# jesselasse/MARL-DMFB

Hardware: AMD Instinct MI355X
Metric: env-steps/sec (whole node), 10x10 DMFB 4-droplet fov9 (higher is better)
Workload: dtype int8 env state/obs + f64 rewards; fp32 Q-net

## Files before the change

__graft_entry__.py:

```python
import os
import subprocess
import sys

ROOT = os.path.dirname(os.path.abspath(__file__))
if ROOT not in sys.path:
    sys.path.insert(0, ROOT)


def build():
    jobs = str(max(1, min(8, os.cpu_count() or 1)))
    env = dict(os.environ, PYTORCH_ROCM_ARCH='gfx950')
    subprocess.check_call(['make', '-C', os.path.join(ROOT, 'marl_dmfb_amd', 'csrc'), '-j', jobs, '-s'], env=env)
    subprocess.check_call(['make', '-C', os.path.join(ROOT, 'oracle'), '-s'], env=env)
    import marl_dmfb_amd
    from marl_dmfb_amd import _lib
    lib = _lib.dmfb_vec()
    for name in _lib.DMFB_VEC_SYMBOLS:
        getattr(lib, name)
    lib = _lib.meda_vec()
    for name in _lib.MEDA_VEC_SYMBOLS:
        getattr(lib, name)
    lib = _lib.crnn_ops()
    for name in ('crnn_conv9_forward', 'crnn_front9_forward', 'crnn_front19_forward', 'crnn_front_padded_cols', 'crnn_conv9_backward', 'crnn_conv19_backward', 'crnn_front9_forward_live', 'gru_seq_forward', 'gru_seq_backward', 'gru_seq_forward_packed', 'gru_seq_backward_packed'):
        getattr(lib, name)
    lib = _lib.rollout_ops()
    for name in ('rollout_select_actions', 'rollout_post_step', 'rollout_gru_head_select_stream', 'rollout_stream_step'):
        getattr(lib, name)
    lib = _lib.vdn_ops()
    for name in ('vdn_td_forward', 'vdn_td_backward', 'vdn_td_forward_packed', 'vdn_td_backward_packed', 'vdn_gather_units', 'vdn_clip_adam_step'):
        getattr(lib, name)
    lib = _lib.qmix_ops()
    for name in _lib.SIGNATURES['qmix_ops']:
        getattr(lib, name)


def smoke():
    import numpy as np
    import torch
    from marl_dmfb_amd.env.dmfb import VecDMFB
    from oracle.dmfb_oracle import DmfbOracle

    assert torch.cuda.is_available(), 'smoke() needs the GPU'
    cfg = dict(width=10, length=10, n_agents=4, fov=9)
    E, seed = 256, 1234
    env = VecDMFB(n_envs=E, seed=seed, device='cuda:0', **cfg)
    ora = DmfbOracle(n_envs=E, seed=seed, **cfg)
    env.reset()
    ora.reset()
    rng = np.random.default_rng(0)
    for t in range(50):
        a = rng.integers(0, 5, (E, 4)).astype(np.int32)
        obs, r, d, info = env.step(torch.as_tensor(a, device='cuda:0'), autoreset=True)
        ro, do, co, so = ora.step(a)
        term = do.all(axis=1)
        if term.any():
            ora.reset(mask=term.astype(np.uint8))
        assert np.array_equal(r.cpu().numpy().view(np.int64), ro.view(np.int64)), 'rewards differ at step %d' % t
        assert np.array_equal(d.cpu().numpy(), do), 'dones differ at step %d' % t
        assert np.array_equal(info['constraints'].cpu().numpy(), co)
        assert np.array_equal(info['success'].cpu().numpy(), so)
        assert np.array_equal(obs.cpu().numpy(), ora.observe()), 'obs differ at step %d' % t
    from marl_dmfb_amd.env.meda import VecMEDA
    from oracle.meda_oracle import MedaOracle
    mcfg = dict(width=30, length=30, n_agents=4, fov=19)
    menv = VecMEDA(n_envs=64, seed=seed, device='cuda:0', **mcfg)
    mora = MedaOracle(n_envs=64, seed=seed, **mcfg)
    menv.reset()
    mora.reset()
    for t in range(30):
        a = rng.integers(0, 9, (64, 4)).astype(np.int32)
        obs, r, d, info = menv.step(torch.as_tensor(a, device='cuda:0'), autoreset=True)
        ro, do, fo, so = mora.step(a)
        term = do.all(axis=1)
        if term.any():
            mora.reset(mask=term.astype(np.uint8))
        assert np.array_equal(r.cpu().numpy().view(np.int64), ro.view(np.int64)), 'MEDA rewards differ at step %d' % t
        assert np.array_equal(d.cpu().numpy(), do) and np.array_equal(obs.cpu().numpy(), mora.observe()), 'MEDA step %d' % t
    print('smoke ok: DMFB %d envs x 50 and MEDA 64 envs x 30 lock-step transitions bit-exact vs CPU oracle' % E)


if __name__ == '__main__':
    build()
    if len(sys.argv) > 1 and sys.argv[1] == 'smoke':
        smoke()
```

marl_dmfb_amd/_lib.py:

```python
import ctypes as C
import os

_HERE = os.path.dirname(os.path.abspath(__file__))
LIB_DIR = os.path.join(_HERE, 'lib')
_CACHE = {}


class HipLibraryMissing(RuntimeError):
    pass


def load(name):
    if name in _CACHE:
        return _CACHE[name]
    path = os.path.join(LIB_DIR, 'lib%s%s.so' % (name, os.environ.get('MARL_DMFB_VARIANT_' + name.upper(), '')))
    if not os.path.exists(path):
        raise HipLibraryMissing(
            '%s not found: build the HIP extension first (python -c "import __graft_entry__ as g; g.build()" '
            'or make -C marl_dmfb_amd/csrc). There is no CPU fallback.' % path)
    import torch
    lib = C.CDLL(path)
    _CACHE[name] = lib
    return lib


class DmfbVecConfig(C.Structure):
    _fields_ = [('width', C.c_int32), ('length', C.c_int32), ('n_agents', C.c_int32), ('n_blocks', C.c_int32),
                ('fov', C.c_int32), ('stall', C.c_int32), ('b_degrade', C.c_int32), ('with_maps', C.c_int32),
                ('per_degrade', C.c_double), ('n_envs', C.c_int32), ('env_id0', C.c_uint32), ('seed', C.c_uint64),
                ('device', C.c_int32)]


class DmfbVecStepOut(C.Structure):
    _fields_ = [('d_rewards', C.c_void_p), ('d_dones', C.c_void_p), ('d_constraints', C.c_void_p),
                ('d_success', C.c_void_p), ('d_obs', C.c_void_p), ('d_team_reward', C.c_void_p),
                ('d_terminated', C.c_void_p), ('d_obs_terminal', C.c_void_p)]


class MedaVecConfig(C.Structure):
    _fields_ = [('width', C.c_int32), ('length', C.c_int32), ('n_agents', C.c_int32), ('fov', C.c_int32),
                ('b_degrade', C.c_int32), ('with_maps', C.c_int32), ('per_degrade', C.c_double), ('n_envs', C.c_int32),
                ('env_id0', C.c_uint32), ('seed', C.c_uint64), ('device', C.c_int32), ('obs_version', C.c_int32)]


class MedaVecStepOut(C.Structure):
    _fields_ = [('d_rewards', C.c_void_p), ('d_dones', C.c_void_p), ('d_fail', C.c_void_p), ('d_success', C.c_void_p),
                ('d_obs', C.c_void_p), ('d_team_reward', C.c_void_p), ('d_terminated', C.c_void_p)]


class RolloutStage(C.Structure):
    _fields_ = [('d_t_ep', C.c_void_p), ('d_o0', C.c_void_p), ('d_o_next', C.c_void_p), ('d_u', C.c_void_p),
                ('d_onehot', C.c_void_p), ('d_r', C.c_void_p), ('d_ep_acc', C.c_void_p), ('d_chip_acc', C.c_void_p),
                ('d_close_slot', C.c_void_p), ('d_state_alt', C.c_void_p)]


class RolloutRing(C.Structure):
    _fields_ = [('slots', C.c_int32), ('d_o', C.c_void_p), ('d_o_next', C.c_void_p), ('d_u', C.c_void_p),
                ('d_u_onehot', C.c_void_p), ('d_avail_u', C.c_void_p), ('d_avail_u_next', C.c_void_p), ('d_r', C.c_void_p),
                ('d_padded', C.c_void_p), ('d_terminated', C.c_void_p), ('d_len', C.c_void_p), ('d_stats', C.c_void_p),
                ('d_state', C.c_void_p)]


class QmixMixer(C.Structure):
    _fields_ = [('w1', C.c_void_p), ('b1', C.c_void_p), ('w2', C.c_void_p), ('b2', C.c_void_p), ('wb', C.c_void_p),
                ('bb', C.c_void_p)]


vp, i32, u32, i64, u64, f32, f64 = C.c_void_p, C.c_int32, C.c_uint32, C.c_int64, C.c_uint64, C.c_float, C.c_double
_dmfb_cfg, _meda_cfg = C.POINTER(DmfbVecConfig), C.POINTER(MedaVecConfig)
_i32p, _f64p = C.POINTER(C.c_int32), C.POINTER(C.c_double)

SIGNATURES = {
    'dmfb_vec': {
        'dmfb_vec_check_config': [_dmfb_cfg],
        'dmfb_vec_create': [_dmfb_cfg, vp, C.POINTER(vp)],
        'dmfb_vec_destroy': [vp],
        'dmfb_vec_state_bytes': ([vp], C.c_size_t),
        'dmfb_vec_obs_len': ([vp], i32),
        'dmfb_vec_max_step': ([vp], i32),
        'dmfb_vec_n_envs': ([vp], i32),
        'dmfb_vec_n_agents': ([vp], i32),
        'dmfb_vec_reset': [vp, vp, i32, vp, vp],
        'dmfb_vec_restart': [vp, vp, vp, vp],
        'dmfb_vec_set_task': [vp, vp, vp, vp],
        'dmfb_vec_get_task': [vp, vp, vp, vp],
        'dmfb_vec_set_blocks': [vp, vp, i32, vp],
        'dmfb_vec_get_blocks': [vp, vp, _i32p, vp],
        'dmfb_vec_step': [vp, vp, vp, vp, u32, C.POINTER(DmfbVecStepOut), vp],
        'dmfb_vec_observe': [vp, vp, vp, vp],
        'dmfb_vec_get_state': [vp, vp, vp, vp, vp, vp],
        'dmfb_vec_state_len': ([vp], i32),
        'dmfb_vec_global_obs': [vp, vp, vp, vp],
        'dmfb_vec_global_obs_append': [vp, vp, vp, i32, i32, vp, vp, vp],
        'dmfb_vec_get_map': [vp, i32, vp, vp],
        'dmfb_vec_set_map': [vp, i32, vp, vp],
        'dmfb_vec_launch_shape': [vp, C.POINTER(C.c_int32 * 6)],
        'dmfb_vec_observe_timing': [vp, i32],
        'dmfb_vec_observe_timing_read': [vp, _f64p, _i32p],
        'dmfb_vec_zoom_lut': [vp, vp],
        'dmfb_vec_strerror': ([i32], C.c_char_p),
        'dmfb_vec_last_hip_error': ([], i32),
    },
    'meda_vec': {
        'meda_vec_check_config': [_meda_cfg],
        'meda_vec_create': [_meda_cfg, vp, C.POINTER(vp)],
        'meda_vec_destroy': [vp],
        'meda_vec_state_bytes': ([vp], C.c_size_t),
        'meda_vec_obs_len': ([vp], i32),
        'meda_vec_max_step': ([vp], i32),
        'meda_vec_n_envs': ([vp], i32),
        'meda_vec_n_agents': ([vp], i32),
        'meda_vec_reset': [vp, vp, vp, vp],
        'meda_vec_restart': [vp, vp, vp, vp],
        'meda_vec_set_task': [vp, vp, vp, vp],
        'meda_vec_get_task': [vp, vp, vp, vp],
        'meda_vec_step': [vp, vp, vp, vp, u32, C.POINTER(MedaVecStepOut), vp],
        'meda_vec_observe': [vp, vp, vp, vp],
        'meda_vec_get_state': [vp, vp, vp, vp, vp, vp],
        'meda_vec_get_map': [vp, i32, vp, vp],
        'meda_vec_set_map': [vp, i32, vp, vp],
        'meda_vec_launch_shape': [vp, C.POINTER(C.c_int32 * 4)],
        'meda_vec_observe_timing': [vp, i32],
        'meda_vec_observe_timing_read': [vp, _f64p, _i32p],
        'meda_vec_strerror': ([i32], C.c_char_p),
        'meda_vec_last_hip_error': ([], i32),
    },
    'crnn_ops': {
        'crnn_conv9_forward': [vp, i64, i64, vp, vp, vp, vp, i32, vp, i64, vp],
        'crnn_front9_forward': [vp, i64, vp, i32, i64, vp, vp, vp, vp, vp, vp, i32, vp, i64, i32, vp],
        'crnn_front9_forward_live': [vp, i64, vp, i32, i64, vp, vp, vp, vp, vp, vp, i32, vp, i64, i32, vp, vp, i32, vp],
        'crnn_front19_forward': [vp, i64, vp, i32, i64, vp, vp, vp, vp, vp, vp, i32, vp, i64, i32, vp],
        'crnn_front_padded_cols': ([i32], i32),
        'crnn_conv9_backward_parts': ([i32], i32),
        'crnn_conv9_backward': [vp, i64, i64, vp, i64, vp, i64, vp, vp, vp, i32, vp, i32, vp, vp],
        'crnn_mlp_backward_parts': ([], i32),
        'crnn_mlp_backward': [vp, i64, i32, vp, i32, i64, vp, i64, vp, i64, i32, vp, vp, vp, vp],
        'crnn_conv19_backward_parts': ([i32], i32),
        'crnn_conv19_backward': [vp, i64, i64, vp, i64, vp, i64, vp, vp, vp, vp, i32, vp, i32, vp, vp],
        'crnn_last_hip_error': ([], i32),
        'gru_seq_forward': [vp, vp, vp, vp, vp, i32, i64, i32, vp, vp, vp],
        'gru_seq_backward': [vp, vp, vp, vp, vp, i32, i64, i32, vp, vp, vp, vp, vp],
        'gru_seq_forward_packed': [vp, vp, vp, vp, vp, i32, i64, i32, _i32p, vp, vp, vp],
        'gru_seq_forward_packed_pair': [vp] * 14 + [i32, i64, i32, _i32p, vp],
        'gru_seq_backward_packed': [vp, vp, vp, vp, vp, i32, i64, i32, _i32p, vp, vp, vp, vp, vp, vp],
        'gru_seq_row_blocks': ([i64], i64),
        'gru_last_hip_error': ([], i32),
    },
    'rollout_ops': {
        'rollout_select_actions': [vp, i32, i32, i32, vp, i32, u64, vp, vp, vp, vp, vp, i32, i32, vp],
        'rollout_gru_head_select': [vp, vp, vp, vp, vp, vp, vp, i32, i32, i32, i32, vp, i32, u64, vp, vp, vp, vp, vp, i32, i32, vp, vp],
        'rollout_gru_head_select_live': [vp, vp, vp, vp, vp, vp, vp, i32, i32, i32, i32, vp, i32, u64, vp, vp, vp, vp, vp, i32, i32, vp, vp,
                                         vp, vp],
        'rollout_compact_alive': [i32, vp, vp, vp, vp],
        'rollout_post_step': [i32, i32, i32, vp, vp, vp, vp, i32, vp, vp, vp, vp, vp, vp, vp, vp, vp, f32, f32, vp, vp, vp, i32, vp, vp,
                              vp],
        'rollout_gru_head_select_stream': [vp, vp, vp, vp, vp, vp, vp, i32, i32, i32, i32, vp, i32, u64, vp, vp, vp, vp, vp, i32, vp, vp,
                                           vp],
        'rollout_stream_step': [i32, i32, i32, i32, i32, i32, vp, vp, vp, vp, vp, vp, i32, vp, C.POINTER(RolloutStage),
                                C.POINTER(RolloutRing), i32, vp, vp, vp, f32, f32, vp, vp],
        'rollout_last_hip_error': ([], i32),
    },
    'vdn_ops': {
        'vdn_td_forward': [vp, vp, vp, vp, vp, vp, vp, i32, i32, i32, i32, i32, f32, vp, vp, vp, vp],
        'vdn_td_backward': [vp, vp, vp, vp, i32, i32, i32, i32, i32, vp, vp],
        'vdn_td_forward_packed': [vp, vp, vp, i32, vp, vp, vp, vp, vp, i32, i32, f32, vp, vp, vp, vp],
        'vdn_td_backward_packed': [vp, vp, vp, i32, vp, vp, i32, i32, vp, vp],
        'vdn_gather_units': [vp, i32, vp, i32, i32, i32, vp, vp],
        'vdn_clip_adam_step': [i32, C.POINTER(vp), C.POINTER(vp), C.POINTER(vp), C.POINTER(vp), C.POINTER(i64), f32, f64, f64, f64,
                               f64, f64, f64, vp, vp, vp, vp],
        'vdn_last_hip_error': ([], i32),
    },
    'qmix_ops': {
        'qmix_mix_td_forward': [vp, vp, vp, vp, vp, vp, vp, i32, i32, i32, i32, i32, vp, i32, i32, vp, i32, i32, i32, i32,
                                C.POINTER(QmixMixer), C.POINTER(QmixMixer), f32, vp, vp, vp, vp],
        'qmix_mix_td_backward': [vp, vp, vp, vp, i32, i32, i32, i32, i32, vp, i32, i32, i32, i32, C.POINTER(QmixMixer), vp, vp, vp,
                                 vp, vp, vp],
        'qmix_last_hip_error': ([], i32),
    },
}

DMFB_VEC_SYMBOLS = list(SIGNATURES['dmfb_vec'])
MEDA_VEC_SYMBOLS = list(SIGNATURES['meda_vec'])

ENV_ERRORS = {
    'dmfb_vec': {
        -1: (ValueError, 'bad argument'),
        -2: (RuntimeError, 'Fov is too large'),
        -3: (TypeError, 'Too many droplets for DMFB'),
        -4: (AssertionError, 'width >= 5 and length >= 5'),
        -5: (AssertionError, 'n_agents > 0'),
        -6: (NotImplementedError, 'configuration outside the build limits (include/dmfb_vec.h)'),
        -7: (TypeError, 'action is illegal'),
        -8: (RuntimeError, 'env was created without health/usage/degrade maps (pass with_maps=True)'),
    },
    'meda_vec': {
        -1: (ValueError, 'bad argument'),
        -3: (RuntimeError, 'Too many droplets in the MEDA array'),
        -4: (AssertionError, 'w > 0 and l > 0'),
        -5: (AssertionError, 'n_agents > 0'),
        -6: (NotImplementedError, 'configuration outside the build limits (include/meda_vec.h)'),
        -8: (RuntimeError, 'env was created without health/usage/degrade maps (pass with_maps=True)'),
    },
}
HIP_ERROR = -100
_LAST_ERROR = {'dmfb_vec_': 'dmfb_vec_last_hip_error', 'meda_vec_': 'meda_vec_last_hip_error', 'crnn_': 'crnn_last_hip_error',
               'gru_': 'gru_last_hip_error', 'rollout_': 'rollout_last_hip_error', 'vdn_': 'vdn_last_hip_error',
               'qmix_': 'qmix_last_hip_error'}


def _typed(lib, name):
    for fn, sig in SIGNATURES[name].items():
        f = getattr(lib, fn)
        if isinstance(sig, tuple):
            f.argtypes, f.restype = sig
        else:
            f.argtypes = sig
    return lib


def _raiser(name, lib):
    errors = ENV_ERRORS.get(name)

    def errcheck(rc, func, args):
        if rc == 0:
            return rc
        fn = func.__name__
        last = getattr(lib, _LAST_ERROR[next(p for p in _LAST_ERROR if fn.startswith(p))])
        if errors is None:
            raise RuntimeError('%s failed: %d (hip %d)' % (fn, rc, last()))
        if rc == HIP_ERROR:
            raise RuntimeError('HIP runtime error %d in %s' % (last(), name))
        exc, msg = errors.get(rc, (RuntimeError, '%s error %d' % (name, rc)))
        raise exc(msg)
    return errcheck


def _library(name):
    lib = load(name)
    if not getattr(lib, '_typed', False):
        _typed(lib, name)
        lib._typed = True
    return lib


def checked(name):
    key = name + ':checked'
    if key not in _CACHE:
        raw = _library(name)
        lib = _typed(C.CDLL(raw._name), name)
        errcheck = _raiser(name, raw)
        for fn, sig in SIGNATURES[name].items():
            if not isinstance(sig, tuple):
                getattr(lib, fn).errcheck = errcheck
        _CACHE[key] = lib
    return _CACHE[key]


def dmfb_vec():
    return _library('dmfb_vec')


def meda_vec():
    return _library('meda_vec')


def crnn_ops():
    return _library('crnn_ops')


def rollout_ops():
    return _library('rollout_ops')


def vdn_ops():
    return _library('vdn_ops')


def qmix_ops():
    return _library('qmix_ops')
```

marl_dmfb_amd/csrc/crnn_ops.hip:

```cpp
#include <hip/hip_runtime.h>

#include <cstdint>
#include <cstdio>
#include <cstdlib>

#include "../../include/crnn_ops.h"

#define HIP_ABI_TAG "crnn_ops"
#define HIP_ABI_ERR CRNN_ERR_HIP
#include "hip_abi.h"
#include "crnn_mfma.h"
#include "crnn_mfma19.h"
#include "crnn_bwd19.h"

namespace {

constexpr int kBlock = 512;
constexpr int kA1Stride = 52;
constexpr int kDz1Unit = 108;

constexpr int kLdsBudget = 158 * 1024;

template <int OD> struct GeoB {
    static constexpr int DZ2 = 28;
    static constexpr int DZ_ROW = OD * DZ2 + 4;
    static constexpr int ROW_FLOATS = OD * kA1Stride + OD * DZ2 + 4 + 244 + (OD / 2) * kDz1Unit;
    static constexpr int FIXED_FLOATS = OD * OD * 9;
    static constexpr int RBB = ((kLdsBudget / 4 - FIXED_FLOATS) / ROW_FLOATS) < (kBlock / (2 * OD)) ? ((kLdsBudget / 4 - FIXED_FLOATS) / ROW_FLOATS)
                                                                                                   : (kBlock / (2 * OD));
    static constexpr size_t LDS_FLOATS = (size_t)FIXED_FLOATS + (size_t)RBB * ROW_FLOATS + OD * 28;
    static constexpr int UNITS = OD * (OD / 2);
    static constexpr int NA = UNITS >= kBlock ? kBlock : kBlock / 2;
    static constexpr int NB = UNITS - NA;
    static constexpr int XSLICES = NB > 0 ? (kBlock - NA) / NB : 1;
    static_assert(NB >= 0 && (NB == 0 || (NA + NB * XSLICES <= kBlock && XSLICES <= 8)), "dW2 roles");
    static constexpr int ITEMS3 = (OD / 2) * 9;
    static constexpr int RS3 = kBlock / ITEMS3;
    static constexpr int PART = kBlock * 9 + kBlock * 9 + OD + kBlock * 6 + OD;
};

template <int OD>
__global__ __launch_bounds__(kBlock) void k_conv9_bwd(const int8_t *__restrict__ obs, long obs_stride, long rows,
                                                      const float *__restrict__ a2, long a2_stride, const float *__restrict__ g, long g_stride,
                                                      const float *__restrict__ w2, float *__restrict__ part,
                                                      const float *__restrict__ w1, const float *__restrict__ b1) {
    using G = GeoB<OD>;
    extern __shared__ __attribute__((aligned(16))) float lds[];
    float *s_w2 = lds;
    float *s_a1 = s_w2 + OD * OD * 9;
    float *s_dz2 = s_a1 + G::RBB * OD * kA1Stride;
    float *s_in = s_dz2 + G::RBB * G::DZ_ROW;
    float *s_dz1 = s_in + G::RBB * 244;
    float *s_w1 = s_dz1 + G::RBB * (OD / 2) * kDz1Unit;
    const int tid = threadIdx.x;
    for (int i = tid; i < OD * 27; i += kBlock) s_w1[i] = w1[i];
    if (tid < OD) s_w1[OD * 27 + tid] = b1[tid];
    for (int i = tid; i < OD * OD * 9; i += kBlock) {
        const int c2 = i / (OD * 9), rem = i - c2 * OD * 9, c1 = rem / 9, tap = rem - c1 * 9;
        s_w2[(c2 * 9 + tap) * OD + c1] = w2[i];
    }
    float accB2 = 0.0f, accB1 = 0.0f, accB1y = 0.0f;
    float2 accW2[9], accW1[3];
#pragma unroll
    for (int k = 0; k < 9; ++k) accW2[k] = make_float2(0.0f, 0.0f);
#pragma unroll
    for (int k = 0; k < 3; ++k) accW1[k] = make_float2(0.0f, 0.0f);
    const bool pa_full = tid < G::NA;
    const int pa_unit = pa_full ? tid : G::NA + (G::NB > 0 ? (tid - G::NA) % (G::NB > 0 ? G::NB : 1) : 0);
    const int pa_slice = pa_full ? 0 : (G::NB > 0 ? (tid - G::NA) / (G::NB > 0 ? G::NB : 1) : 0);
    const bool pa_on = pa_full || (G::NB > 0 && pa_slice < G::XSLICES);
    const int pa_step = pa_full ? 1 : G::XSLICES;
    const int pa_c2 = pa_unit / (OD / 2), pa_cp = pa_unit - pa_c2 * (OD / 2);
    const int i3 = tid % G::ITEMS3, s3 = tid / G::ITEMS3;
    const bool p3_on = s3 < G::RS3;
    const int cp_3 = i3 / 9, c0_3 = (i3 - cp_3 * 9) / 3, kx_3 = i3 - cp_3 * 9 - c0_3 * 3;

    constexpr int kSplit2 = G::NB > 0 ? 2 : 4, kBase2 = G::NB > 0 ? kBlock / 2 : 0;
    const int q2 = (tid - kBase2) & (kSplit2 - 1), unit2 = tid >= kBase2 ? (tid - kBase2) / kSplit2 : G::RBB * (OD / 2);
    const int r2 = unit2 / (OD / 2), cp2 = unit2 - r2 * (OD / 2);
    const int br = tid / OD, bc = tid - br * OD;

    const long n_blocks = (rows + G::RBB - 1) / G::RBB;
    const long per = (n_blocks + gridDim.x - 1) / gridDim.x;
    const long blk0 = (long)blockIdx.x * per, blk1 = min(n_blocks, blk0 + per);

    typedef float f32x4 __attribute__((ext_vector_type(4)));
    const int lane = tid & 63, wave = tid >> 6, j16 = lane & 15, kq = lane >> 4;
    const int c_nh = (wave >> 1) & 1, c_sub = (wave & 1) + 2 * (wave >> 2), c_ch = c_nh * 16 + j16;
    const bool c_chv = c_ch < OD;
    constexpr int NPD = (G::RBB * OD * 25 + kBlock - 1) / kBlock, NPI = (G::RBB * 243 + kBlock - 1) / kBlock;
    float pfa[NPD], pfg[NPD];
    int pfi[NPI];
#pragma unroll
    for (int u = 0; u < NPD; ++u) { pfa[u] = 0.0f; pfg[u] = 0.0f; }
#pragma unroll
    for (int u = 0; u < NPI; ++u) pfi[u] = 0;
    auto fetch = [&](long b) {
        const long r0 = b * G::RBB;
        const int rvb = b < blk1 ? (int)min((long)G::RBB, rows - r0) : 0;
        if (rvb <= 0) return;
        int t_ = tid;
        asm volatile("" : "+v"(t_));
#pragma unroll
        for (int u = 0; u < NPD; ++u) {
            const int i = min(t_ + u * kBlock, G::RBB * OD * 25 - 1), rr = i / (OD * 25), rem = i - rr * OD * 25;
            const long row = r0 + min(rr, rvb - 1);
            pfa[u] = a2[row * a2_stride + rem];
            pfg[u] = g[row * g_stride + rem];
        }
#pragma unroll
        for (int u = 0; u < NPI; ++u) {
            const int i = min(t_ + u * kBlock, G::RBB * 243 - 1), rr = i / 243, pp = i - rr * 243;
            pfi[u] = obs[(r0 + min(rr, rvb - 1)) * obs_stride + pp];
        }
    };
    fetch(blk0);
    for (long blk = blk0; blk < blk1; ++blk) {
        const long row0 = blk * G::RBB;
        const int rv = (int)min((long)G::RBB, rows - row0);
        __syncthreads();
        int t_ = tid;
        asm volatile("" : "+v"(t_));
#pragma unroll
        for (int u = 0; u < NPD; ++u) {
            const int i = t_ + u * kBlock, rc = i / 25, k = i - rc * 25;
            if (i < G::RBB * OD * 25) s_dz2[(rc / OD) * G::DZ_ROW + (rc % OD) * G::DZ2 + k] = (rc / OD < rv && pfa[u] > 0.0f) ? pfg[u] : 0.0f;
        }
#pragma unroll
        for (int u = 0; u < NPI; ++u) {
            const int i = t_ + u * kBlock, rr = i / 243, pp = i - rr * 243;
            if (i < G::RBB * 243) s_in[rr * 244 + pp] = rr < rv ? (float)pfi[u] : 0.0f;
        }
        __syncthreads();
        int off1[7], goff[3];
        float bw1[7];
        int kq_ = kq, j_ = j16;
        asm volatile("" : "+v"(kq_), "+v"(j_));
#pragma unroll
        for (int s = 0; s < 7; ++s) {
            const int k = 4 * s + kq_, c0 = k / 9, tap = k - c0 * 9;
            off1[s] = k < 27 ? c0 * 81 + (tap / 3) * 9 + tap % 3 : 0;
            const float w = s_w1[(c_chv ? c_ch : 0) * 27 + (k < 27 ? k : 0)];
            bw1[s] = (c_chv && k < 27) ? w : 0.0f;
        }
        const float c_bias = c_chv ? s_w1[OD * 27 + c_ch] : 0.0f;
#pragma unroll
        for (int qt = 0; qt < 3; ++qt) { const int p = qt * 16 + j_; goff[qt] = (p / 7) * 9 + p % 7; }
        for (int rr = c_sub; rr < G::RBB; rr += 4) {
            float cv[3][7];
#pragma unroll
            for (int qt = 0; qt < 3; ++qt)
#pragma unroll
                for (int s = 0; s < 7; ++s) cv[qt][s] = s_in[rr * 244 + goff[qt] + off1[s]];
            f32x4 acc[3];
#pragma unroll
            for (int qt = 0; qt < 3; ++qt) acc[qt] = f32x4{c_bias, c_bias, c_bias, c_bias};
#pragma unroll
            for (int s = 0; s < 7; ++s)
#pragma unroll
                for (int qt = 0; qt < 3; ++qt) acc[qt] = __builtin_amdgcn_mfma_f32_16x16x4f32(cv[qt][s], bw1[s], acc[qt], 0, 0, 0);
            if (c_chv) {
                float *dst = s_a1 + ((rr * (OD / 2) + (c_ch >> 1)) * kA1Stride + kq * 4) * 2 + (c_ch & 1);
#pragma unroll
                for (int qt = 0; qt < 3; ++qt)
#pragma unroll
                    for (int q = 0; q < 4; ++q) dst[(qt * 16 + q) * 2] = fmaxf(acc[qt][q], 0.0f);
            }
        }
        if (c_sub == 0) {
            const int rr = j16 < G::RBB ? j16 : G::RBB - 1;
            f32x4 acc = {c_bias, c_bias, c_bias, c_bias};
#pragma unroll
            for (int s = 0; s < 7; ++s) acc = __builtin_amdgcn_mfma_f32_16x16x4f32(s_in[rr * 244 + 60 + off1[s]], bw1[s], acc, 0, 0, 0);
            if (c_chv) {
#pragma unroll
                for (int q = 0; q < 4; ++q)
                    if (kq * 4 + q < G::RBB) s_a1[(((kq * 4 + q) * (OD / 2) + (c_ch >> 1)) * kA1Stride + 48) * 2 + (c_ch & 1)] = fmaxf(acc[q], 0.0f);
            }
        }
        __syncthreads();
        auto unit_rows = [&](int c2, int cp, int r_begin, int r_step) {
#pragma unroll 1
            for (int rr = r_begin; rr < rv; rr += r_step) {
                float dz[G::DZ2];
                float2 a[kA1Stride];
                const float4 *pd = (const float4 *)__builtin_assume_aligned(s_dz2 + rr * G::DZ_ROW + c2 * G::DZ2, 16);
                const float4 *pa = (const float4 *)__builtin_assume_aligned(s_a1 + (size_t)(rr * (OD / 2) + cp) * 2 * kA1Stride, 16);
#pragma unroll
                for (int j = 0; j < G::DZ2 / 4; ++j) { const float4 t = pd[j]; dz[4 * j] = t.x; dz[4 * j + 1] = t.y; dz[4 * j + 2] = t.z; dz[4 * j + 3] = t.w; }
#pragma unroll
                for (int j = 0; j < kA1Stride / 2; ++j) { const float4 t = pa[j]; a[2 * j] = make_float2(t.x, t.y); a[2 * j + 1] = make_float2(t.z, t.w); }
#pragma unroll
                for (int kx = 0; kx < 3; ++kx)
#pragma unroll
                    for (int ky = 0; ky < 3; ++ky)
#pragma unroll
                        for (int x = 0; x < 5; ++x)
#pragma unroll
                            for (int y = 0; y < 5; ++y) {
                                const float z = dz[x * 5 + y];
                                const float2 v = a[(x + kx) * 7 + y + ky];
                                accW2[kx * 3 + ky].x = fmaf(z, v.x, accW2[kx * 3 + ky].x);
                                accW2[kx * 3 + ky].y = fmaf(z, v.y, accW2[kx * 3 + ky].y);
                            }
            }
        };
        if (tid < G::RBB * OD && br < rv) {
            const float4 *pd = (const float4 *)__builtin_assume_aligned(s_dz2 + br * G::DZ_ROW + bc * G::DZ2, 16);
            float t = 0.0f;
#pragma unroll
            for (int j = 0; j < 6; ++j) { const float4 v = pd[j]; t += (v.x + v.y) + (v.z + v.w); }
            accB2 += t + pd[6].x;
        }
#ifndef CRNN_PROBE_SKIP_P1
        if (pa_on) unit_rows(pa_c2, pa_cp, pa_slice, pa_step);
#endif
#ifndef CRNN_PROBE_SKIP_P2
        const bool p2 = unit2 < G::RBB * (OD / 2) && r2 < rv;
#else
        const bool p2 = false;
#endif
        if (p2) {
            float2 da[49];
#pragma unroll
            for (int k = 0; k < 49; ++k) da[k] = make_float2(0.0f, 0.0f);
            const int cbeg = q2 * (OD / kSplit2), cend = cbeg + OD / kSplit2;
#pragma unroll 1
            for (int c2 = cbeg; c2 < cend; ++c2) {
                float dz[G::DZ2];
                float2 w[9];
                const float4 *pd = (const float4 *)__builtin_assume_aligned(s_dz2 + r2 * G::DZ_ROW + c2 * G::DZ2, 16);
#pragma unroll
                for (int j = 0; j < G::DZ2 / 4; ++j) { const float4 t = pd[j]; dz[4 * j] = t.x; dz[4 * j + 1] = t.y; dz[4 * j + 2] = t.z; dz[4 * j + 3] = t.w; }
#pragma unroll
                for (int k = 0; k < 9; ++k) w[k] = *(const float2 *)(s_w2 + (c2 * 9 + k) * OD + 2 * cp2);
#pragma unroll
                for (int kx = 0; kx < 3; ++kx)
#pragma unroll
                    for (int ky = 0; ky < 3; ++ky)
#pragma unroll
                        for (int x = 0; x < 5; ++x)
#pragma unroll
                            for (int y = 0; y < 5; ++y) {
                                float2 &d = da[(x + kx) * 7 + y + ky];
                                const float z = dz[x * 5 + y];
                                d.x = fmaf(z, w[kx * 3 + ky].x, d.x);
                                d.y = fmaf(z, w[kx * 3 + ky].y, d.y);
                            }
            }
#ifndef CRNN_PROBE_P2_NO_DPP
#pragma unroll
            for (int k = 0; k < 49; ++k) {
                asm volatile("v_add_f32_dpp %0, %0, %0 quad_perm:[1,0,3,2] row_mask:0xf bank_mask:0xf bound_ctrl:1" : "+v"(da[k].x));
                asm volatile("v_add_f32_dpp %0, %0, %0 quad_perm:[1,0,3,2] row_mask:0xf bank_mask:0xf bound_ctrl:1" : "+v"(da[k].y));
            }
            if (kSplit2 == 4) {
                asm volatile("s_nop 1");
#pragma unroll
                for (int k = 0; k < 49; ++k) {
                    asm volatile("v_add_f32_dpp %0, %0, %0 quad_perm:[2,3,0,1] row_mask:0xf bank_mask:0xf bound_ctrl:1" : "+v"(da[k].x));
                    asm volatile("v_add_f32_dpp %0, %0, %0 quad_perm:[2,3,0,1] row_mask:0xf bank_mask:0xf bound_ctrl:1" : "+v"(da[k].y));
                }
            }
#endif
#ifdef CRNN_PROBE_P2_NO_MASK
            if (q2 == 0 && da[0].x == 12345.678f) {
#else
            if (q2 == 0) {
#endif
                const float4 *act = (const float4 *)__builtin_assume_aligned(s_a1 + (size_t)unit2 * 2 * kA1Stride, 16);
                unsigned long long lx = 0, ly = 0;
#pragma unroll
                for (int j = 0; j < 25; ++j) {
                    const float4 a = act[j];
                    lx |= (unsigned long long)((a.x > 0.0f ? 1u : 0u) | (a.z > 0.0f ? 2u : 0u)) << (2 * j);
                    ly |= (unsigned long long)((a.y > 0.0f ? 1u : 0u) | (a.w > 0.0f ? 2u : 0u)) << (2 * j);
                }
                float4 *dst4 = (float4 *)__builtin_assume_aligned(s_dz1 + (size_t)unit2 * kDz1Unit, 16);
                float sx = 0.0f, sy = 0.0f;
#pragma unroll
                for (int j = 0; j < 25; ++j) {
                    float4 o;
                    o.x = (lx >> (2 * j)) & 1 ? da[2 * j].x : 0.0f;
                    o.y = (ly >> (2 * j)) & 1 ? da[2 * j].y : 0.0f;
                    o.z = (2 * j + 1 < 49 && ((lx >> (2 * j + 1)) & 1)) ? da[2 * j + 1 < 49 ? 2 * j + 1 : 0].x : 0.0f;
                    o.w = (2 * j + 1 < 49 && ((ly >> (2 * j + 1)) & 1)) ? da[2 * j + 1 < 49 ? 2 * j + 1 : 0].y : 0.0f;
                    dst4[j] = o;
                    sx += o.x + o.z;
                    sy += o.y + o.w;
                }
                accB1 += sx;
                accB1y += sy;
            }
        }
        __syncthreads();
        fetch(blk + 1);
#ifdef CRNN_PROBE_SKIP_P3
        if (false) {
#else
        if (p3_on) {
#endif
            for (int rr = s3; rr < rv; rr += G::RS3) {
                const float2 *pd = (const float2 *)(s_dz1 + (size_t)(rr * (OD / 2) + cp_3) * kDz1Unit);
                const float *in = s_in + rr * 244 + c0_3 * 81 + kx_3 * 9;
#pragma unroll
                for (int x = 0; x < 7; ++x) {
                    float2 dz[7];
                    float v[9];
#pragma unroll
                    for (int y = 0; y < 7; ++y) dz[y] = pd[x * 7 + y];
#pragma unroll
                    for (int y = 0; y < 9; ++y) v[y] = in[x * 9 + y];
#pragma unroll
                    for (int ky = 0; ky < 3; ++ky)
#pragma unroll
                        for (int y = 0; y < 7; ++y) {
                            typedef float f32x2 __attribute__((ext_vector_type(2)));
                            const f32x2 r = __builtin_elementwise_fma((f32x2){dz[y].x, dz[y].y}, (f32x2){v[y + ky], v[y + ky]},
                                                                      (f32x2){accW1[ky].x, accW1[ky].y});
                            accW1[ky] = make_float2(r.x, r.y);
                        }
                }
            }
        }
    }
    __syncthreads();
    if (tid < G::RBB * OD) s_dz2[OD * 16 + bc * 16 + br] = accB2;
    if (q2 == 0 && unit2 < G::RBB * (OD / 2)) {
        s_dz2[(2 * cp2) * 16 + r2] = accB1;
        s_dz2[(2 * cp2 + 1) * 16 + r2] = accB1y;
    }
    __syncthreads();
    float *pp = part + (size_t)blockIdx.x * G::PART;
#pragma unroll
    for (int k = 0; k < 9; ++k) { pp[tid * 18 + 2 * k] = accW2[k].x; pp[tid * 18 + 2 * k + 1] = accW2[k].y; }
    if (tid < OD) {
        float t = 0.0f;
        for (int k = 0; k < G::RBB; ++k) t += s_dz2[OD * 16 + tid * 16 + k];
        pp[kBlock * 18 + tid] = t;
    }
#pragma unroll
    for (int k = 0; k < 3; ++k) { pp[kBlock * 18 + OD + tid * 6 + k] = accW1[k].x; pp[kBlock * 18 + OD + tid * 6 + 3 + k] = accW1[k].y; }
    if (tid < OD) {
        float t = 0.0f;
        for (int k = 0; k < G::RBB; ++k) t += s_dz2[tid * 16 + k];
        pp[kBlock * 18 + OD + kBlock * 6 + tid] = t;
    }
}

constexpr int kRedY = 16;
template <int OD>
__global__ __launch_bounds__(64 * kRedY) void k_conv9_bwd_reduce(const float *__restrict__ part, int n_part, float *__restrict__ grads) {
    using G = GeoB<OD>;
    __shared__ float s_sum[kRedY][64];
    const int tx = threadIdx.x & 63, ty = threadIdx.x >> 6;
    const int i = blockIdx.x * 64 + tx;
    const int n2 = OD * OD * 9, nb = OD, n1 = OD * 27;
    float acc = 0.0f;
    if (i < n2 + nb + n1 + nb) {
        int off[8], cnt = 0;
        if (i < n2) {
            const int pair = i / 9, tap = i - pair * 9, c2 = pair / OD, c1 = pair - c2 * OD;
            const int unit = c2 * (OD / 2) + (c1 >> 1), comp = 2 * tap + (c1 & 1);
            if (unit < G::NA) off[cnt++] = unit * 18 + comp;
            else
                for (int sl = 0; sl < G::XSLICES && sl < 8; ++sl) off[cnt++] = (G::NA + sl * G::NB + (unit - G::NA)) * 18 + comp;
        } else if (i < n2 + nb) {
            off[cnt++] = kBlock * 18 + (i - n2);
        } else if (i < n2 + nb + n1) {
            const int jx = i - n2 - nb, c1 = jx / 27, r = jx - c1 * 27, ky = r % 3;
            const int item = (c1 >> 1) * 9 + r / 3;
            for (int sl = 0; sl < G::RS3; ++sl) off[cnt++] = kBlock * 18 + OD + (sl * G::ITEMS3 + item) * 6 + (c1 & 1) * 3 + ky;
        } else {
            off[cnt++] = kBlock * 18 + OD + kBlock * 6 + (i - n2 - nb - n1);
        }
        for (int k = 0; k < cnt; ++k) {
            float a0 = 0.0f, a1 = 0.0f;
            int b = ty;
            for (; b + kRedY < n_part; b += 2 * kRedY) { a0 += part[(size_t)b * G::PART + off[k]]; a1 += part[(size_t)(b + kRedY) * G::PART + off[k]]; }
            if (b < n_part) a0 += part[(size_t)b * G::PART + off[k]];
            acc += a0 + a1;
        }
    }
    s_sum[ty][tx] = acc;
    __syncthreads();
    if (ty == 0 && i < n2 + nb + n1 + nb) {
        float t = 0.0f;
#pragma unroll
        for (int k = 0; k < kRedY; ++k) t += s_sum[k][tx];
        grads[i] = t;
    }
}

constexpr int kMlpBlock = 256, kMlpOut = 10, kMlpMaxIn = 18, kMlpMaxParts = 256;
__global__ __launch_bounds__(kMlpBlock) void k_mlp_bwd(const int8_t *__restrict__ obs, long obs_stride, int dir_off,
                                                       const int8_t *__restrict__ onehot, int n_actions, long rows,
                                                       const float *__restrict__ x, long x_stride, const float *__restrict__ g, long g_stride,
                                                       int col0, float *__restrict__ part) {
    __shared__ float s_red[kMlpBlock / 64][kMlpOut * (kMlpMaxIn + 1)];
    float acc[kMlpOut][kMlpMaxIn + 1];
#pragma unroll
    for (int o = 0; o < kMlpOut; ++o)
#pragma unroll
        for (int k = 0; k <= kMlpMaxIn; ++k) acc[o][k] = 0.0f;
    for (long r = (long)blockIdx.x * kMlpBlock + threadIdx.x; r < rows; r += (long)gridDim.x * kMlpBlock) {
        float v[kMlpMaxIn];
        v[0] = (float)obs[r * obs_stride + dir_off];
        v[1] = (float)obs[r * obs_stride + dir_off + 1];
#pragma unroll
        for (int k = 0; k < kMlpMaxIn - 2; ++k) v[2 + k] = k < n_actions ? (float)onehot[r * n_actions + k] : 0.0f;
#pragma unroll
        for (int o = 0; o < kMlpOut; ++o) {
            const float gz = x[r * x_stride + col0 + o] > 0.0f ? g[r * g_stride + col0 + o] : 0.0f;
#pragma unroll
            for (int k = 0; k < kMlpMaxIn; ++k) acc[o][k] = fmaf(gz, v[k], acc[o][k]);
            acc[o][kMlpMaxIn] += gz;
        }
    }
    const int lane = threadIdx.x & 63, wave = threadIdx.x >> 6;
#pragma unroll
    for (int o = 0; o < kMlpOut; ++o)
#pragma unroll
        for (int k = 0; k <= kMlpMaxIn; ++k) {
            float t = acc[o][k];
            for (int d = 32; d > 0; d >>= 1) t += __shfl_xor(t, d);
            if (lane == 0) s_red[wave][o * (kMlpMaxIn + 1) + k] = t;
        }
    __syncthreads();
    for (int i = threadIdx.x; i < kMlpOut * (kMlpMaxIn + 1); i += kMlpBlock) {
        float t = 0.0f;
#pragma unroll
        for (int w = 0; w < kMlpBlock / 64; ++w) t += s_red[w][i];
        part[(size_t)blockIdx.x * kMlpOut * (kMlpMaxIn + 1) + i] = t;
    }
}
__global__ __launch_bounds__(256) void k_mlp_bwd_reduce(const float *__restrict__ part, int n_part, int nin, float *__restrict__ dw, float *__restrict__ db) {
    const int i = threadIdx.x;
    if (i >= kMlpOut * nin + kMlpOut) return;
    const int o = i < kMlpOut * nin ? i / nin : i - kMlpOut * nin, k = i < kMlpOut * nin ? i - o * nin : kMlpMaxIn;
    float t = 0.0f;
    for (int b = 0; b < n_part; ++b) t += part[(size_t)b * kMlpOut * (kMlpMaxIn + 1) + o * (kMlpMaxIn + 1) + k];
    if (i < kMlpOut * nin) dw[i] = t;
    else db[o] = t;
}

struct LiveRows { const int32_t *chips; const int32_t *n; int rows_per_chip; };

template <int OD, int RBV>
int launch_rb(const int8_t *obs, long obs_stride, long rows, const float *w1, const float *b1, const float *w2, const float *b2,
              float *out, long out_stride, int out_cols, const int8_t *onehot, int n_actions, const float *mlp_w, const float *mlp_b, hipStream_t s,
              LiveRows live = LiveRows{nullptr, nullptr, 1}) {
    using GM = crnn_mfma::GeoM<OD, RBV>;
    const size_t lds = GM::LDS_FLOATS * sizeof(float);
    static LdsLimit lds_limit;
    if (const int rc = lds_limit.raise((const void *)crnn_mfma::k_conv9_mfma<OD, RBV>, lds)) return rc;
    const long n_blocks = (rows + GM::RB - 1) / GM::RB;
    const long resident = 256L * (long)((size_t)160 * 1024 / lds);
    const int grid = (int)(n_blocks < resident ? n_blocks : resident);
    LAUNCH((crnn_mfma::k_conv9_mfma<OD, RBV>), dim3(grid), dim3(crnn_mfma::kBlockM), lds, s, obs, obs_stride, rows, w1, b1, w2, b2,
           out, out_stride, out_cols, onehot, n_actions, mlp_w, mlp_b, live.chips, live.n, live.rows_per_chip);
    return CRNN_OK;
}

template <int OD>
int launch(const int8_t *obs, long obs_stride, long rows, const float *w1, const float *b1, const float *w2, const float *b2,
           float *out, long out_stride, int out_cols, const int8_t *onehot, int n_actions, const float *mlp_w, const float *mlp_b, hipStream_t s,
           LiveRows live = LiveRows{nullptr, nullptr, 1}) {
    return launch_rb<OD, 0>(obs, obs_stride, rows, w1, b1, w2, b2, out, out_stride, out_cols, onehot, n_actions, mlp_w, mlp_b, s, live);
}

template <int OD>
int launch19(const int8_t *obs, long obs_stride, long rows, const float *w1, const float *b1, const float *w3, const float *b3,
             float *out, long out_stride, int out_cols, const int8_t *onehot, int n_actions, const float *mlp_w, const float *mlp_b, hipStream_t s) {
    using GM = crnn_mfma19::Geo<OD>;
    const size_t lds = GM::LDS_FLOATS * sizeof(float);
    static LdsLimit lds_limit;
    if (const int rc = lds_limit.raise((const void *)crnn_mfma19::k_conv19_mfma<OD>, lds)) return rc;
    const long n_blocks = (rows + GM::RB - 1) / GM::RB;
    const int grid = (int)(n_blocks < 256 ? n_blocks : 256);
    LAUNCH((crnn_mfma19::k_conv19_mfma<OD>), dim3(grid), dim3(crnn_mfma19::kBlockM), lds, s, obs, obs_stride, rows, w1, b1, w3,
           b3, out, out_stride, out_cols, onehot, n_actions, mlp_w, mlp_b);
    return CRNN_OK;
}

template <int OD>
int launch_bwd(const int8_t *obs, long obs_stride, long rows, const float *a2, long a2_stride,
               const float *g, long g_stride, const float *w2, float *part, int grid, float *grads, const float *w1, const float *b1,
               hipStream_t s) {
    using G = GeoB<OD>;
    const size_t lds = G::LDS_FLOATS * sizeof(float);
    static LdsLimit lds_limit;
    if (const int rc = lds_limit.raise((const void *)k_conv9_bwd<OD>, lds)) return rc;
    HIP_TRY(launch_status([&] {
        hipLaunchKernelGGL((k_conv9_bwd<OD>), dim3(grid), dim3(kBlock), lds, s, obs, obs_stride, rows, a2, a2_stride, g, g_stride,
                           w2, part, w1, b1);
        const int n_out = OD * OD * 9 + OD + OD * 27 + OD;
        hipLaunchKernelGGL((k_conv9_bwd_reduce<OD>), dim3((n_out + 63) / 64), dim3(64 * kRedY), 0, s, part, grid, grads);
    }));
    return CRNN_OK;
}

template <int OD>
int launch_bwd19(const int8_t *obs, long obs_stride, long rows, const float *a3, long a3_stride, const float *g, long g_stride,
                 const float *w1, const float *b1, const float *w3, const float *b3, float *part, int n_part, float *grads, hipStream_t s) {
    using G = crnn_bwd19::GeoB19<OD>;
    const size_t lds = G::LDS_FLOATS * sizeof(float);
    static LdsLimit lds_limit;
    if (const int rc = lds_limit.raise((const void *)crnn_bwd19::k_conv19_bwd<OD>, lds)) return rc;
    const long n_blocks = (rows + G::RBB - 1) / G::RBB;
    const int grid = (int)(n_blocks < n_part ? n_blocks : n_part);
    HIP_TRY(launch_status([&] {
        hipLaunchKernelGGL((crnn_bwd19::k_conv19_bwd<OD>), dim3(grid), dim3(crnn_bwd19::kBlockB), lds, s, obs, obs_stride, rows, a3, a3_stride, g,
                           g_stride, w1, b1, w3, b3, part);
        hipLaunchKernelGGL((crnn_bwd19::k_conv19_bwd_reduce<OD>), dim3((G::GRADS + 63) / 64), dim3(64 * crnn_bwd19::kRedY19), 0, s, part, grid, grads);
    }));
    return CRNN_OK;
}

}

extern "C" {

int crnn_conv9_forward(const int8_t *d_obs, int64_t obs_stride, int64_t rows, const float *d_w1, const float *d_b1,
                       const float *d_w2, const float *d_b2, int od, float *d_out, int64_t out_stride, void *stream) {
    if (!d_obs || !d_w1 || !d_b1 || !d_w2 || !d_b2 || !d_out || rows < 0 || obs_stride < 243 || out_stride < od * 25)
        return CRNN_ERR_BAD_ARG;
    if (rows == 0) return CRNN_OK;
    if (od == 24) return launch<24>(d_obs, obs_stride, rows, d_w1, d_b1, d_w2, d_b2, d_out, out_stride, 0, nullptr, 0, nullptr, nullptr, (hipStream_t)stream);
    if (od == 32) return launch<32>(d_obs, obs_stride, rows, d_w1, d_b1, d_w2, d_b2, d_out, out_stride, 0, nullptr, 0, nullptr, nullptr, (hipStream_t)stream);
    return CRNN_ERR_UNSUPPORTED;
}

int crnn_front9_forward(const int8_t *d_obs, int64_t obs_stride, const int8_t *d_onehot, int n_actions, int64_t rows,
                        const float *d_w1, const float *d_b1, const float *d_w2, const float *d_b2, const float *d_mlp_w,
                        const float *d_mlp_b, int od, float *d_out, int64_t out_stride, int out_cols, void *stream) {
    if (!d_obs || !d_w1 || !d_b1 || !d_w2 || !d_b2 || !d_mlp_w || !d_mlp_b || !d_out || rows < 0 || obs_stride < 245 ||
        out_stride < od * 25 + 10 || n_actions < 0 || n_actions > 16)
        return CRNN_ERR_BAD_ARG;
    if (od != 24 && od != 32) return CRNN_ERR_UNSUPPORTED;
    if (out_cols != 0 && (out_cols < od * 25 + 10 || out_cols > crnn_front_padded_cols(od) || out_cols > out_stride)) return CRNN_ERR_BAD_ARG;
    if (rows == 0) return CRNN_OK;
    if (od == 24) return launch<24>(d_obs, obs_stride, rows, d_w1, d_b1, d_w2, d_b2, d_out, out_stride, out_cols, d_onehot, n_actions, d_mlp_w, d_mlp_b, (hipStream_t)stream);
    return launch<32>(d_obs, obs_stride, rows, d_w1, d_b1, d_w2, d_b2, d_out, out_stride, out_cols, d_onehot, n_actions, d_mlp_w, d_mlp_b, (hipStream_t)stream);
}

int crnn_front9_forward_live(const int8_t *d_obs, int64_t obs_stride, const int8_t *d_onehot, int n_actions, int64_t rows,
                             const float *d_w1, const float *d_b1, const float *d_w2, const float *d_b2, const float *d_mlp_w,
                             const float *d_mlp_b, int od, float *d_out, int64_t out_stride, int out_cols, const int32_t *d_live_chips,
                             const int32_t *d_n_live, int rows_per_chip, void *stream) {
    if (!d_obs || !d_w1 || !d_b1 || !d_w2 || !d_b2 || !d_mlp_w || !d_mlp_b || !d_out || rows < 0 || obs_stride < 245 ||
        out_stride < od * 25 + 10 || n_actions < 0 || n_actions > 16 || !d_live_chips || !d_n_live || rows_per_chip < 1 ||
        rows_per_chip > 64 || rows % rows_per_chip != 0 || rows >= (1 << 25))
        return CRNN_ERR_BAD_ARG;
    if (od != 24 && od != 32) return CRNN_ERR_UNSUPPORTED;
    if (out_cols != 0 && (out_cols < od * 25 + 10 || out_cols > crnn_front_padded_cols(od) || out_cols > out_stride)) return CRNN_ERR_BAD_ARG;
    if (rows == 0) return CRNN_OK;
    const LiveRows live{d_live_chips, d_n_live, rows_per_chip};
    if (od == 24) return launch<24>(d_obs, obs_stride, rows, d_w1, d_b1, d_w2, d_b2, d_out, out_stride, out_cols, d_onehot, n_actions, d_mlp_w, d_mlp_b, (hipStream_t)stream, live);
    return launch<32>(d_obs, obs_stride, rows, d_w1, d_b1, d_w2, d_b2, d_out, out_stride, out_cols, d_onehot, n_actions, d_mlp_w, d_mlp_b, (hipStream_t)stream, live);
}

int crnn_front_padded_cols(int od) { return od == 24 ? crnn_mfma::GeoM<24>::PAD_COLS : od == 32 ? crnn_mfma::GeoM<32>::PAD_COLS : CRNN_ERR_UNSUPPORTED; }

int crnn_front19_forward(const int8_t *d_obs, int64_t obs_stride, const int8_t *d_onehot, int n_actions, int64_t rows,
                         const float *d_w1, const float *d_b1, const float *d_w3, const float *d_b3, const float *d_mlp_w,
                         const float *d_mlp_b, int od, float *d_out, int64_t out_stride, int out_cols, void *stream) {
    const bool vec = d_mlp_w != nullptr;
    const int n_feat = od * 25 + (vec ? 10 : 0);
    if (!d_obs || !d_w1 || !d_b1 || !d_w3 || !d_b3 || !d_out || rows < 0 || obs_stride < 3 * 19 * 19 + (vec ? 2 : 0) ||
        out_stride < n_feat || n_actions < 0 || n_actions > 16 || (vec && !d_mlp_b))
        return CRNN_ERR_BAD_ARG;
    if (od != 24 && od != 32) return CRNN_ERR_UNSUPPORTED;
    if (out_cols != 0 && (out_cols < n_feat || out_cols > crnn_front_padded_cols(od) || out_cols > out_stride)) return CRNN_ERR_BAD_ARG;
    if (rows == 0) return CRNN_OK;
    if (od == 24) return launch19<24>(d_obs, obs_stride, rows, d_w1, d_b1, d_w3, d_b3, d_out, out_stride, out_cols, d_onehot, n_actions, d_mlp_w, d_mlp_b, (hipStream_t)stream);
    return launch19<32>(d_obs, obs_stride, rows, d_w1, d_b1, d_w3, d_b3, d_out, out_stride, out_cols, d_onehot, n_actions, d_mlp_w, d_mlp_b, (hipStream_t)stream);
}

int crnn_conv9_backward_parts(int od) { return od == 24 ? GeoB<24>::PART : od == 32 ? GeoB<32>::PART : CRNN_ERR_UNSUPPORTED; }

int crnn_conv9_backward(const int8_t *d_obs, int64_t obs_stride, int64_t rows, const float *d_out, int64_t out_stride,
                        const float *d_grad_out, int64_t grad_stride, const float *d_w1, const float *d_b1, const float *d_w2,
                        int od, float *d_part, int n_part, float *d_grads, void *stream) {
    if (!d_obs || !d_out || !d_grad_out || !d_w1 || !d_b1 || !d_w2 || !d_part || !d_grads || rows <= 0 || n_part < 1 || n_part > 256)
        return CRNN_ERR_BAD_ARG;
    if (od == 24) return launch_bwd<24>(d_obs, obs_stride, rows, d_out, out_stride, d_grad_out, grad_stride, d_w2, d_part, n_part, d_grads, d_w1, d_b1, (hipStream_t)stream);
    if (od == 32) return launch_bwd<32>(d_obs, obs_stride, rows, d_out, out_stride, d_grad_out, grad_stride, d_w2, d_part, n_part, d_grads, d_w1, d_b1, (hipStream_t)stream);
    return CRNN_ERR_UNSUPPORTED;
}

int crnn_mlp_backward_parts(void) { return kMlpMaxParts * kMlpOut * (kMlpMaxIn + 1); }

int crnn_mlp_backward(const int8_t *d_obs, int64_t obs_stride, int dir_offset, const int8_t *d_onehot, int n_actions, int64_t rows,
                      const float *d_out, int64_t out_stride, const float *d_grad_out, int64_t grad_stride, int col0, float *d_part,
                      float *d_grad_w, float *d_grad_b, void *stream) {
    if (!d_obs || !d_onehot || !d_out || !d_grad_out || !d_part || !d_grad_w || !d_grad_b || rows <= 0 || n_actions < 0 ||
        n_actions > kMlpMaxIn - 2 || dir_offset < 0 || obs_stride < dir_offset + 2 || col0 < 0 || out_stride < col0 + kMlpOut ||
        grad_stride < col0 + kMlpOut)
        return CRNN_ERR_BAD_ARG;
    const long want = (rows + kMlpBlock - 1) / kMlpBlock;
    const int grid = (int)(want < kMlpMaxParts ? want : kMlpMaxParts);
    HIP_TRY(launch_status([&] {
        hipLaunchKernelGGL(k_mlp_bwd, dim3(grid), dim3(kMlpBlock), 0, (hipStream_t)stream, d_obs, (long)obs_stride, dir_offset, d_onehot, n_actions,
                           (long)rows, d_out, (long)out_stride, d_grad_out, (long)grad_stride, col0, d_part);
        hipLaunchKernelGGL(k_mlp_bwd_reduce, dim3(1), dim3(256), 0, (hipStream_t)stream, d_part, grid, 2 + n_actions, d_grad_w, d_grad_b);
    }));
    return CRNN_OK;
}

int crnn_conv19_backward_parts(int od) { return od == 24 ? crnn_bwd19::GeoB19<24>::PART : od == 32 ? crnn_bwd19::GeoB19<32>::PART : CRNN_ERR_UNSUPPORTED; }

int crnn_conv19_backward(const int8_t *d_obs, int64_t obs_stride, int64_t rows, const float *d_out, int64_t out_stride,
                         const float *d_grad_out, int64_t grad_stride, const float *d_w1, const float *d_b1, const float *d_w3,
                         const float *d_b3, int od, float *d_part, int n_part, float *d_grads, void *stream) {
    if (!d_obs || !d_out || !d_grad_out || !d_w1 || !d_b1 || !d_w3 || !d_b3 || !d_part || !d_grads || rows <= 0 || n_part < 1 ||
        n_part > 256 || obs_stride < 3 * 19 * 19 || out_stride < od * 25 || grad_stride < od * 25)
        return CRNN_ERR_BAD_ARG;
    if (od == 24) return launch_bwd19<24>(d_obs, obs_stride, rows, d_out, out_stride, d_grad_out, grad_stride, d_w1, d_b1, d_w3, d_b3, d_part, n_part, d_grads, (hipStream_t)stream);
    if (od == 32) return launch_bwd19<32>(d_obs, obs_stride, rows, d_out, out_stride, d_grad_out, grad_stride, d_w1, d_b1, d_w3, d_b3, d_part, n_part, d_grads, (hipStream_t)stream);
    return CRNN_ERR_UNSUPPORTED;
}

int crnn_last_hip_error(void) { return g_last_hip; }

}
```

marl_dmfb_amd/network/base_net.py:

```python
import os

import torch
import torch.nn as nn
import torch.nn.functional as f


_CONV_PLAN = {5: [(True, 1)], 7: [(True, 1), (False, 1)], 9: [(True, 1), (False, 1)], 11: [(True, 1), (False, 1)],
              13: [(True, 1), (False, 1)], 19: [(True, 2), (False, 1), (False, 1)]}


class _ConvGemm(torch.autograd.Function):

    @staticmethod
    def forward(ctx, cols, weight2d, bias):
        ctx.save_for_backward(cols, weight2d)
        return torch.addmm(bias, cols, weight2d.t())

    @staticmethod
    def backward(ctx, g):
        cols, w = ctx.saved_tensors
        g = g.contiguous()
        gcols = g @ w if ctx.needs_input_grad[0] else None
        M, K = cols.shape
        C = g.shape[1]
        S = 1
        while S < 512 and M % (S * 2) == 0 and M // (S * 2) >= 1024:
            S *= 2
        gw = torch.bmm(g.view(S, M // S, C).transpose(1, 2), cols.view(S, M // S, K)).sum(0)
        return gcols, gw, _colsum(g)


N_PART = 256


def _conv9_backward(obs_i8, x, g, w1c, b1c, w2c, od):
    from .. import _lib
    lib = _lib.checked('crnn_ops')
    if g.stride(1) != 1:
        g = g.contiguous()
    R = obs_i8.shape[0]
    tot = torch.empty(od * od * 9 + od + od * 27 + od, dtype=torch.float32, device=g.device)
    part = torch.empty((N_PART, lib.crnn_conv9_backward_parts(od)), dtype=torch.float32, device=g.device)
    lib.crnn_conv9_backward(obs_i8.data_ptr(), obs_i8.stride(0), R, x.data_ptr(), x.stride(0), g.data_ptr(),
                            g.stride(0), w1c.data_ptr(), b1c.data_ptr(), w2c.data_ptr(), od, part.data_ptr(),
                            N_PART, tot.data_ptr(), torch.cuda.current_stream(g.device).cuda_stream)
    return tot


def _mlp_branch_backward(obs_i8, dir_off, onehot_i8, x, g, col0):
    from .. import _lib
    lib = _lib.checked('crnn_ops')
    A = onehot_i8.shape[1]
    if g.stride(1) != 1:
        g = g.contiguous()
    g_w = torch.empty((10, 2 + A), dtype=torch.float32, device=g.device)
    g_b = torch.empty((10,), dtype=torch.float32, device=g.device)
    part = torch.empty((lib.crnn_mlp_backward_parts(),), dtype=torch.float32, device=g.device)
    lib.crnn_mlp_backward(obs_i8.data_ptr(), obs_i8.stride(0), dir_off, onehot_i8.data_ptr(), A, obs_i8.shape[0],
                          x.data_ptr(), x.stride(0), g.data_ptr(), g.stride(0), col0, part.data_ptr(),
                          g_w.data_ptr(), g_b.data_ptr(), torch.cuda.current_stream(g.device).cuda_stream)
    return g_w, g_b


class _ConvFront9(torch.autograd.Function):

    @staticmethod
    def forward(ctx, obs_i8, w1, b1, w2, b2):
        from .. import _lib
        lib = _lib.checked('crnn_ops')
        obs_i8 = obs_i8.contiguous()
        R, od = obs_i8.shape[0], w1.shape[0]
        out = torch.empty((R, od * 25), dtype=torch.float32, device=obs_i8.device)
        w1c, b1c, w2c, b2c = (t.detach().contiguous() for t in (w1, b1, w2, b2))
        lib.crnn_conv9_forward(obs_i8.data_ptr(), obs_i8.stride(0), R, w1c.data_ptr(), b1c.data_ptr(),
                               w2c.data_ptr(), b2c.data_ptr(), od, out.data_ptr(), out.stride(0),
                               torch.cuda.current_stream(obs_i8.device).cuda_stream)
        ctx.save_for_backward(obs_i8, out, w1c, b1c, w2c)
        ctx.shapes = (w1.shape, w2.shape)
        return out

    @staticmethod
    def backward(ctx, g):
        obs_i8, out, w1c, b1c, w2c = ctx.saved_tensors
        (s1, s2) = ctx.shapes
        od = s1[0]
        n2 = od * od * 9
        tot = _conv9_backward(obs_i8, out, g, w1c, b1c, w2c, od)
        return None, tot[n2 + od:n2 + od + od * 27].view(s1), tot[n2 + od + od * 27:], tot[:n2].view(s2), tot[n2:n2 + od]


class _Front9Train(torch.autograd.Function):

    @staticmethod
    def forward(ctx, obs_i8, onehot_i8, w1, b1, w2, b2, mlp_w, mlp_b, cols):
        from .. import _lib
        lib = _lib.checked('crnn_ops')
        obs_i8, onehot_i8 = obs_i8.contiguous(), onehot_i8.contiguous()
        R, od, A = obs_i8.shape[0], w1.shape[0], onehot_i8.shape[1]
        x = torch.empty((R, cols), dtype=torch.float32, device=obs_i8.device)
        w1c, b1c, w2c, b2c, mwc, mbc = (t.detach().contiguous() for t in (w1, b1, w2, b2, mlp_w, mlp_b))
        lib.crnn_front9_forward(obs_i8.data_ptr(), obs_i8.stride(0), onehot_i8.data_ptr(), A, R, w1c.data_ptr(),
                                b1c.data_ptr(), w2c.data_ptr(), b2c.data_ptr(), mwc.data_ptr(),
                                mbc.data_ptr(), od, x.data_ptr(), x.stride(0), cols,
                                torch.cuda.current_stream(obs_i8.device).cuda_stream)
        ctx.save_for_backward(obs_i8, onehot_i8, x, w1c, b1c, w2c)
        ctx.shapes = (w1.shape, w2.shape)
        return x

    @staticmethod
    def backward(ctx, g):
        obs_i8, onehot_i8, x, w1c, b1c, w2c = ctx.saved_tensors
        (s1, s2) = ctx.shapes
        od = s1[0]
        n2 = od * od * 9
        tot = _conv9_backward(obs_i8, x, g, w1c, b1c, w2c, od)
        g_mw, g_mb = _mlp_branch_backward(obs_i8, 243, onehot_i8, x, g, od * 25)
        return (None, None, tot[n2 + od:n2 + od + od * 27].view(s1), tot[n2 + od + od * 27:], tot[:n2].view(s2), tot[n2:n2 + od],
                g_mw, g_mb, None)


class _Front19Train(torch.autograd.Function):

    @staticmethod
    def forward(ctx, obs_i8, onehot_i8, w1, b1, w3, b3, mlp_w, mlp_b, cols):
        from .. import _lib
        lib = _lib.checked('crnn_ops')
        obs_i8, onehot_i8 = obs_i8.contiguous(), onehot_i8.contiguous()
        R, od, A = obs_i8.shape[0], w1.shape[0], onehot_i8.shape[1]
        x = torch.empty((R, cols), dtype=torch.float32, device=obs_i8.device)
        w1c, b1c, w3c, b3c, mwc, mbc = (t.detach().contiguous() for t in (w1, b1, w3, b3, mlp_w, mlp_b))
        lib.crnn_front19_forward(obs_i8.data_ptr(), obs_i8.stride(0), onehot_i8.data_ptr(), A, R, w1c.data_ptr(),
                                 b1c.data_ptr(), w3c.data_ptr(), b3c.data_ptr(), mwc.data_ptr(),
                                 mbc.data_ptr(), od, x.data_ptr(), x.stride(0), cols,
                                 torch.cuda.current_stream(obs_i8.device).cuda_stream)
        ctx.save_for_backward(obs_i8, onehot_i8, x, w1c, b1c, w3c, b3c)
        ctx.shapes = (w1.shape, w3.shape)
        return x

    @staticmethod
    def backward(ctx, g):
        from .. import _lib
        lib = _lib.checked('crnn_ops')
        obs_i8, onehot_i8, x, w1c, b1c, w3c, b3c = ctx.saved_tensors
        (s1, s3) = ctx.shapes
        od = s1[0]
        if g.stride(1) != 1:
            g = g.contiguous()
        R = obs_i8.shape[0]
        n3 = od * od * 9
        tot = torch.empty(n3 + od + od * 27 + od, dtype=torch.float32, device=g.device)
        part = torch.empty((N_PART, lib.crnn_conv19_backward_parts(od)), dtype=torch.float32, device=g.device)
        lib.crnn_conv19_backward(obs_i8.data_ptr(), obs_i8.stride(0), R, x.data_ptr(), x.stride(0), g.data_ptr(),
                                 g.stride(0), w1c.data_ptr(), b1c.data_ptr(), w3c.data_ptr(), b3c.data_ptr(), od,
                                 part.data_ptr(), N_PART, tot.data_ptr(), torch.cuda.current_stream(g.device).cuda_stream)
        g_mw, g_mb = _mlp_branch_backward(obs_i8, 1083, onehot_i8, x, g, od * 25)
        return (None, None, tot[n3 + od:n3 + od + od * 27].view(s1), tot[n3 + od + od * 27:], tot[:n3].view(s3), tot[n3:n3 + od],
                g_mw, g_mb, None)


class _LinearSplitK(torch.autograd.Function):

    @staticmethod
    def forward(ctx, x, weight, bias):
        ctx.save_for_backward(x, weight)
        ctx.has_bias = bias is not None
        return torch.addmm(bias, x, weight.t()) if bias is not None else torch.matmul(x, weight.t())

    @staticmethod
    def backward(ctx, g):
        x, w = ctx.saved_tensors
        g = g.contiguous()
        gx = torch.matmul(g, w) if ctx.needs_input_grad[0] else None
        return gx, _wgrad_splitk(g, x), (_colsum(g) if ctx.has_bias else None)


def _colsum(t2d):
    M = t2d.shape[0]
    for cand in (256, 128, 64, 32):
        if M % cand == 0 and M // cand >= 64:
            return t2d.reshape(cand, M // cand, -1).sum(1).sum(0)
    return t2d.sum(0)


def _wgrad_splitk(g2d, x2d):
    M = g2d.shape[0]
    S = 1
    for cand in (64, 32, 16, 8, 4, 2):
        if M % cand == 0 and M // cand >= 512:
            S = cand
            break
    if S == 1:
        return torch.matmul(g2d.t(), x2d)
    return torch.bmm(g2d.view(S, M // S, -1).transpose(1, 2), x2d.view(S, M // S, -1)).sum(0)


class _GRUSeq(torch.autograd.Function):

    @staticmethod
    def forward(ctx, igates, h0, w_hh, b_ih, b_hh):
        T = igates.shape[0]
        w_hh_t = w_hh.t()
        h, hs, wss = h0, [], []
        for t in range(T):
            h, ws = torch.ops.aten._thnn_fused_gru_cell(igates[t], torch.matmul(h, w_hh_t), h, b_ih, b_hh)
            hs.append(h)
            wss.append(ws)
        out = torch.stack(hs, dim=0)
        ctx.save_for_backward(out, h0, w_hh, *wss)
        return out

    @staticmethod
    def backward(ctx, grad_out):
        out, h0, w_hh, *wss = ctx.saved_tensors
        T, R, H = out.shape
        d_ig = torch.empty((T, R, 3 * H), dtype=out.dtype, device=out.device)
        d_hg = torch.empty_like(d_ig)
        gh = None
        for t in range(T - 1, -1, -1):
            g = grad_out[t] if gh is None else grad_out[t] + gh
            gi, ghg, ghx, _, _ = torch.ops.aten._thnn_fused_gru_cell_backward(g.contiguous(), wss[t], False)
            d_ig[t] = gi
            d_hg[t] = ghg
            gh = torch.addmm(ghx, ghg, w_hh)
        h_prev = torch.cat([h0.unsqueeze(0), out[:-1]], dim=0)
        d_w_hh = torch.matmul(d_hg.view(T * R, 3 * H).t(), h_prev.view(T * R, H))
        return d_ig, gh, d_w_hh, d_ig.sum(dim=(0, 1)), d_hg.sum(dim=(0, 1))


class _GRUSeqHip(torch.autograd.Function):

    @staticmethod
    def _lib():
        from .. import _lib
        return _lib.checked('crnn_ops')

    @staticmethod
    def run_forward(igates, h0, w_hh, b_ih, b_hh, save):
        lib = _GRUSeqHip._lib()
        T, R, G = igates.shape
        H = G // 3
        igates, h0, w_hh = igates.contiguous(), h0.contiguous(), w_hh.contiguous()
        hs = torch.empty((T, R, H), dtype=torch.float32, device=igates.device)
        gates = torch.empty((T, R, 4 * H), dtype=torch.float32, device=igates.device) if save else None
        lib.gru_seq_forward(igates.data_ptr(), h0.data_ptr(), w_hh.data_ptr(), b_ih.data_ptr(),
                            b_hh.data_ptr(), T, R, H, hs.data_ptr(),
                            gates.data_ptr() if save else None,
                            torch.cuda.current_stream(igates.device).cuda_stream)
        return hs, gates

    @staticmethod
    def forward(ctx, igates, h0, w_hh, b_ih, b_hh):
        hs, gates = _GRUSeqHip.run_forward(igates.detach(), h0.detach(), w_hh.detach(), b_ih.detach(), b_hh.detach(), True)
        ctx.save_for_backward(hs, gates, h0, w_hh)
        return hs

    @staticmethod
    def backward(ctx, grad_out):
        hs, gates, h0, w_hh = ctx.saved_tensors
        lib = _GRUSeqHip._lib()
        T, R, H = hs.shape
        grad_out = grad_out.contiguous()
        h0c, w = h0.contiguous(), w_hh.contiguous()
        d_ig = torch.empty((T, R, 3 * H), dtype=torch.float32, device=hs.device)
        d_hg = torch.empty_like(d_ig)
        d_h0 = torch.empty_like(h0c)
        bias_part = torch.empty((lib.gru_seq_row_blocks(R), 6 * H), dtype=torch.float32, device=hs.device)
        lib.gru_seq_backward(grad_out.data_ptr(), gates.data_ptr(), hs.data_ptr(), h0c.data_ptr(),
                             w.data_ptr(), T, R, H, d_ig.data_ptr(), d_hg.data_ptr(), d_h0.data_ptr(),
                             bias_part.data_ptr(), torch.cuda.current_stream(hs.device).cuda_stream)
        d_w_hh = torch.matmul(d_hg[0].t(), h0c)
        if T > 1:
            d_w_hh = d_w_hh + _wgrad_splitk(d_hg[1:].reshape((T - 1) * R, 3 * H), hs[:-1].reshape((T - 1) * R, H))
        d_b = bias_part.sum(0)
        return d_ig, d_h0, d_w_hh, d_b[:3 * H], d_b[3 * H:]


class _GRUSeqHipPacked(torch.autograd.Function):

    @staticmethod
    def _steps(step_rows):
        import ctypes as C
        return (C.c_int32 * len(step_rows))(*[int(v) for v in step_rows])

    @staticmethod
    def run_forward(igates, h0, w_hh, b_ih, b_hh, step_rows, save):
        lib = _GRUSeqHip._lib()
        Vp, G = igates.shape
        H, T, R, V = G // 3, len(step_rows), h0.shape[0], int(sum(step_rows))
        igates, h0, w_hh = igates.contiguous(), h0.contiguous(), w_hh.contiguous()
        hs = torch.empty((Vp, H), dtype=torch.float32, device=igates.device)
        hs[V:].zero_()
        gates = torch.empty((Vp, 4 * H), dtype=torch.float32, device=igates.device) if save else None
        lib.gru_seq_forward_packed(igates.data_ptr(), h0.data_ptr(), w_hh.data_ptr(), b_ih.data_ptr(),
                                   b_hh.data_ptr(), T, R, H, _GRUSeqHipPacked._steps(step_rows), hs.data_ptr(),
                                   gates.data_ptr() if save else None,
                                   torch.cuda.current_stream(igates.device).cuda_stream)
        return hs, gates

    @staticmethod
    def forward(ctx, igates, h0, w_hh, b_ih, b_hh, step_rows):
        hs, gates = _GRUSeqHipPacked.run_forward(igates.detach(), h0.detach(), w_hh.detach(), b_ih.detach(), b_hh.detach(), step_rows, True)
        ctx.save_for_backward(hs, gates, h0, w_hh)
        ctx.step_rows = list(step_rows)
        return hs

    @staticmethod
    def backward(ctx, grad_out):
        hs, gates, h0, w_hh = ctx.saved_tensors
        lib = _GRUSeqHip._lib()
        step_rows = ctx.step_rows
        Vp, H = hs.shape
        T, R, V = len(step_rows), h0.shape[0], int(sum(step_rows))
        grad_out = grad_out.contiguous()
        h0c, w = h0.contiguous(), w_hh.contiguous()
        d_ig = torch.empty((Vp, 3 * H), dtype=torch.float32, device=hs.device)
        d_hg = torch.empty_like(d_ig)
        h_prev = torch.empty((Vp, H), dtype=torch.float32, device=hs.device)
        for t in (d_ig, d_hg, h_prev):
            t[V:].zero_()
        d_h0 = torch.zeros_like(h0c)
        bias_part = torch.empty((lib.gru_seq_row_blocks(R), 6 * H), dtype=torch.float32, device=hs.device)
        lib.gru_seq_backward_packed(grad_out.data_ptr(), gates.data_ptr(), hs.data_ptr(), h0c.data_ptr(),
                                    w.data_ptr(), T, R, H, _GRUSeqHipPacked._steps(step_rows), d_ig.data_ptr(),
                                    d_hg.data_ptr(), d_h0.data_ptr(), bias_part.data_ptr(), h_prev.data_ptr(),
                                    torch.cuda.current_stream(hs.device).cuda_stream)
        d_w_hh = _wgrad_splitk(d_hg, h_prev)
        d_b = bias_part.sum(0)
        return d_ig, d_h0, d_w_hh, d_b[:3 * H], d_b[3 * H:], None


class _GRUSeqPairPacked(torch.autograd.Function):

    @staticmethod
    def forward(ctx, ig_a, w_hh_a, b_ih_a, b_hh_a, ig_b, w_hh_b, b_ih_b, b_hh_b, step_rows, R):
        lib = _GRUSeqHip._lib()
        Vp, G = ig_a.shape
        Hd, T, V = G // 3, len(step_rows), int(sum(step_rows))
        save = any(ctx.needs_input_grad[:4])
        ta = [t.detach().contiguous() for t in (ig_a, w_hh_a, b_ih_a, b_hh_a)]
        tb = [t.detach().contiguous() for t in (ig_b, w_hh_b, b_ih_b, b_hh_b)]
        hs_a = torch.empty((Vp, Hd), dtype=torch.float32, device=ig_a.device)
        hs_b = torch.empty((Vp, Hd), dtype=torch.float32, device=ig_a.device)
        hs_a[V:].zero_()
        hs_b[V:].zero_()
        gates = torch.empty((Vp, 4 * Hd), dtype=torch.float32, device=ig_a.device) if save else None
        lib.gru_seq_forward_packed_pair(ta[0].data_ptr(), None, ta[1].data_ptr(), ta[2].data_ptr(), ta[3].data_ptr(),
                                        hs_a.data_ptr(), gates.data_ptr() if save else None,
                                        tb[0].data_ptr(), None, tb[1].data_ptr(), tb[2].data_ptr(), tb[3].data_ptr(),
                                        hs_b.data_ptr(), None, T, R, Hd, _GRUSeqHipPacked._steps(step_rows),
                                        torch.cuda.current_stream(ig_a.device).cuda_stream)
        if save:
            h0 = torch.zeros((R, Hd), dtype=torch.float32, device=ig_a.device)
            ctx.save_for_backward(hs_a, gates, h0, ta[1])
            ctx.step_rows = list(step_rows)
        ctx.mark_non_differentiable(hs_b)
        return hs_a, hs_b

    @staticmethod
    def backward(ctx, grad_a, _grad_b):
        d_ig, _d_h0, d_w_hh, d_b_ih, d_b_hh, _ = _GRUSeqHipPacked.backward(ctx, grad_a)
        return d_ig, d_w_hh, d_b_ih, d_b_hh, None, None, None, None, None, None


def gru_sequence(igates, h0, w_hh, b_ih, b_hh, impl='hip'):
    if impl == 'hip' and h0.shape[-1] == 128 and igates.dtype == torch.float32:
        if torch.is_grad_enabled() and any(t.requires_grad for t in (igates, h0, w_hh, b_ih, b_hh)):
            return _GRUSeqHip.apply(igates, h0, w_hh, b_ih, b_hh)
        return _GRUSeqHip.run_forward(igates, h0, w_hh, b_ih, b_hh, False)[0]
    return _GRUSeq.apply(igates, h0, w_hh, b_ih, b_hh)


def conv_str(fov, id=3, od=32):
    stack, shared = [], None
    for from_image, stride in _CONV_PLAN[fov]:
        if from_image:
            stack.append(nn.Conv2d(id, od, kernel_size=3, stride=stride))
        else:
            if shared is None:
                shared = nn.Conv2d(od, od, kernel_size=3, stride=stride)
            stack.append(shared)
    return stack


class CRNN(nn.Module):
    def __init__(self, args):
        super().__init__()
        id = args.obs_shape[0]
        od = args.hyper_hidden_dim
        self.input_dim = tuple(args.obs_shape)
        self.rnn_hidden_dim = args.rnn_hidden_dim
        self.n_actions = args.n_actions
        self.convs = conv_str(args.fov, id, od)
        size = args.fov
        for i, conv in enumerate(self.convs, 1):
            self.add_module('conv{}'.format(i), conv)
            size = int((size + 2 * conv.padding[0] - conv.dilation[0] * (conv.kernel_size[0] - 1) - 1) // conv.stride[0] + 1)
        self.out = size * size * od
        self.n_pixel = self.input_dim[-1] - self.input_dim[-2]
        self.mlp1 = nn.Linear(args.obs_shape[-2] + args.n_actions, 10)
        self.rnn = nn.GRUCell(self.out + 10, args.rnn_hidden_dim)
        self.fc1 = nn.Linear(args.rnn_hidden_dim, args.n_actions)
        self.conv_impl = getattr(args, 'conv_impl', 'gemm')

    def _conv_stack_gemm(self, pixel):
        x = pixel.permute(0, 2, 3, 1)
        for conv in self.convs:
            k, s = conv.kernel_size[0], conv.stride[0]
            win = x.unfold(1, k, s).unfold(2, k, s)
            R, Ho, Wo = win.shape[0], win.shape[1], win.shape[2]
            cols = win.reshape(R * Ho * Wo, -1)
            y = _ConvGemm.apply(cols, conv.weight.view(conv.out_channels, -1), conv.bias)
            x = f.relu(y).view(R, Ho, Wo, conv.out_channels)
        return x.permute(0, 3, 1, 2).reshape(x.shape[0], self.out)

    def features_split(self, pixel, vec):
        pixel = pixel.reshape((-1,) + self.input_dim[:3])
        if pixel.is_cuda and self.conv_impl == 'gemm':
            pixel = self._conv_stack_gemm(pixel)
        else:
            for conv in self.convs:
                pixel = f.relu(conv(pixel))
            pixel = pixel.reshape((-1, self.out))
        vec = f.relu(self.mlp1(vec))
        return torch.cat([pixel, vec], dim=1)

    def features(self, inputs):
        pixel, vec = torch.split(inputs, [self.n_pixel, self.n_actions + self.input_dim[-2]], dim=1)
        return self.features_split(pixel, vec)

    def recurrent(self, x, hidden_state):
        h_in = hidden_state.reshape(-1, self.rnn_hidden_dim)
        h = self.rnn(x, h_in)
        return self.fc1(h), h

    def recurrent_seq(self, x_seq, h0):
        T, R = x_seq.shape[0], x_seq.shape[1]
        h = h0.reshape(-1, self.rnn_hidden_dim)
        hs = []
        if x_seq.is_cuda:
            w_ih = self.weight_ih_padded() if x_seq.shape[-1] == self.padded_cols() != self.rnn.weight_ih.shape[1] else self.rnn.weight_ih
            igates = _LinearSplitK.apply(x_seq.reshape(T * R, -1), w_ih, None).view(T, R, -1)
            hseq = gru_sequence(igates, h, self.rnn.weight_hh, self.rnn.bias_ih, self.rnn.bias_hh,
                                getattr(self, 'gru_impl', 'hip'))
            q = _LinearSplitK.apply(hseq.view(T * R, -1), self.fc1.weight, self.fc1.bias).view(T, R, -1)
            return q, hseq[-1]
        else:
            for t in range(T):
                h = self.rnn(x_seq[t], h)
                hs.append(h)
        q = self.fc1(torch.stack(hs, dim=0).view(T * R, -1)).view(T, R, -1)
        return q, h

    def recurrent_seq_packed(self, x, step_rows, R):
        w_ih = self.weight_ih_padded() if x.shape[-1] == self.padded_cols() != self.rnn.weight_ih.shape[1] else self.rnn.weight_ih
        igates = _LinearSplitK.apply(x, w_ih, None)
        h0 = torch.zeros((R, self.rnn_hidden_dim), dtype=torch.float32, device=x.device)
        args = (igates, h0, self.rnn.weight_hh, self.rnn.bias_ih, self.rnn.bias_hh)
        if torch.is_grad_enabled() and any(t.requires_grad for t in args):
            hs = _GRUSeqHipPacked.apply(*args, step_rows)
        else:
            hs = _GRUSeqHipPacked.run_forward(*args, step_rows, False)[0]
        return _LinearSplitK.apply(hs, self.fc1.weight, self.fc1.bias)

    @staticmethod
    def recurrent_seq_packed_pair(net_a, x_a, net_b, x_b, step_rows, R):
        def w_ih(net, x, grad):
            if x.shape[-1] == net.padded_cols() != net.rnn.weight_ih.shape[1]:
                return net.weight_ih_padded() if grad else net.refresh_padded()
            return net.rnn.weight_ih
        ig_a = _LinearSplitK.apply(x_a, w_ih(net_a, x_a, True), None)
        with torch.no_grad():
            ig_b = torch.matmul(x_b, w_ih(net_b, x_b, False).t())
        hs_a, hs_b = _GRUSeqPairPacked.apply(ig_a, net_a.rnn.weight_hh, net_a.rnn.bias_ih, net_a.rnn.bias_hh,
                                             ig_b, net_b.rnn.weight_hh.detach(), net_b.rnn.bias_ih.detach(), net_b.rnn.bias_hh.detach(),
                                             step_rows, R)
        q_a = _LinearSplitK.apply(hs_a, net_a.fc1.weight, net_a.fc1.bias)
        with torch.no_grad():
            q_b = torch.addmm(net_b.fc1.bias, hs_b, net_b.fc1.weight.t())
        return q_a, q_b

    def forward(self, inputs, hidden_state):
        return self.recurrent(self.features(inputs), hidden_state)

    def _pixel_features_hip(self, obs_i8):
        from .. import _lib
        lib = _lib.checked('crnn_ops')
        obs_i8 = obs_i8.contiguous()
        R = obs_i8.shape[0]
        out = torch.empty((R, self.out), dtype=torch.float32, device=obs_i8.device)
        c1, c2 = self.convs[0], self.convs[1]
        stream = torch.cuda.current_stream(obs_i8.device).cuda_stream
        if self._hip_geometry() == 19:
            lib.crnn_front19_forward(obs_i8.data_ptr(), obs_i8.stride(0), None, 0, R,
                                     c1.weight.data_ptr(), c1.bias.data_ptr(),
                                     c2.weight.data_ptr(), c2.bias.data_ptr(), None, None,
                                     c1.out_channels, out.data_ptr(), out.stride(0), 0, stream)
        else:
            lib.crnn_conv9_forward(obs_i8.data_ptr(), obs_i8.stride(0), R,
                                   c1.weight.data_ptr(), c1.bias.data_ptr(),
                                   c2.weight.data_ptr(), c2.bias.data_ptr(),
                                   c1.out_channels, out.data_ptr(), out.stride(0), stream)
        return out

    def padded_cols(self):
        return (self.out + 10 + 63) // 64 * 64

    def weight_ih_padded(self):
        w = self.rnn.weight_ih
        return f.pad(w, (0, self.padded_cols() - w.shape[1]))

    def refresh_padded(self):
        w = self.rnn.weight_ih.detach()
        buf = getattr(self, '_w_ih_pad', None)
        if buf is None or buf.device != w.device or buf.shape != (w.shape[0], self.padded_cols()):
            buf = self._w_ih_pad = w.new_zeros((w.shape[0], self.padded_cols()))
        buf[:, :w.shape[1]].copy_(w)
        return buf

    def front_features_live(self, obs_i8, onehot_i8, live_chips, n_live, rows_per_chip, out):
        from .. import _lib
        lib = _lib.checked('crnn_ops')
        c1, c2 = self.convs[0], self.convs[1]
        lib.crnn_front9_forward_live(obs_i8.data_ptr(), obs_i8.stride(0), onehot_i8.data_ptr(), self.n_actions, obs_i8.shape[0],
                                     c1.weight.data_ptr(), c1.bias.data_ptr(), c2.weight.data_ptr(), c2.bias.data_ptr(),
                                     self.mlp1.weight.data_ptr(), self.mlp1.bias.data_ptr(), c1.out_channels,
                                     out.data_ptr(), out.stride(0), out.shape[1], live_chips.data_ptr(), n_live.data_ptr(),
                                     int(rows_per_chip), torch.cuda.current_stream(obs_i8.device).cuda_stream)
        return out

    def _front_features_hip(self, obs_i8, onehot_i8, padded=False):
        from .. import _lib
        lib = _lib.checked('crnn_ops')
        obs_i8 = obs_i8.contiguous()
        R = obs_i8.shape[0]
        cols = self.padded_cols() if padded else self.out + 10
        out = torch.empty((R, cols), dtype=torch.float32, device=obs_i8.device)
        c1, c2 = self.convs[0], self.convs[1]
        oh = None
        if onehot_i8 is not None:
            onehot_i8 = onehot_i8.to(torch.int8).contiguous()
            oh = onehot_i8.data_ptr()
        fn = lib.crnn_front19_forward if self._hip_geometry() == 19 else lib.crnn_front9_forward
        fn(obs_i8.data_ptr(), obs_i8.stride(0), oh, self.n_actions, R,
                                c1.weight.data_ptr(), c1.bias.data_ptr(),
                                c2.weight.data_ptr(), c2.bias.data_ptr(),
                                self.mlp1.weight.data_ptr(), self.mlp1.bias.data_ptr(),
                                c1.out_channels, out.data_ptr(), out.stride(0), cols,
                                torch.cuda.current_stream(obs_i8.device).cuda_stream)
        return out

    def features_obs_train(self, obs_i8, la_rows):
        c1, c2 = self.convs[0], self.convs[1]
        if self._hip_geometry() == 19:
            return _Front19Train.apply(obs_i8, la_rows.to(torch.int8), c1.weight, c1.bias, c2.weight, c2.bias,
                                       self.mlp1.weight, self.mlp1.bias, self.padded_cols())
        if self.mlp1.in_features == 2 + self.n_actions and self.n_actions <= 16 and self.mlp1.out_features == 10:
            return _Front9Train.apply(obs_i8, la_rows.to(torch.int8), c1.weight, c1.bias, c2.weight, c2.bias,
                                      self.mlp1.weight, self.mlp1.bias, self.padded_cols())
        pix = _ConvFront9.apply(obs_i8, c1.weight, c1.bias, c2.weight, c2.bias)
        vec = torch.cat([obs_i8[:, self.n_pixel:].float(), la_rows.float()], dim=1)
        return torch.cat([pix, f.relu(self.mlp1(vec))], dim=1)

    def _hip_train_ok(self, obs_i8):
        if not (self.conv_impl == 'gemm' and obs_i8.is_cuda and obs_i8.dtype == torch.int8 and torch.is_grad_enabled()
                and self.convs[0].out_channels in (24, 32)):
            return False
        if self._hip_geometry() == 19:
            return (self.mlp1.in_features == 2 + self.n_actions and self.n_actions <= 16 and self.mlp1.out_features == 10
                    and os.environ.get('MARL_DMFB_CONV19_BWD', '1') != '0')
        return (self.input_dim[:3] == (3, 9, 9) and len(self.convs) == 2 and self.convs[0] is not self.convs[1])

    def _hip_geometry(self):
        cv = self.convs
        if self.input_dim[:3] == (3, 9, 9) and len(cv) == 2 and cv[0] is not cv[1] and cv[0].stride[0] == 1:
            return 9
        if self.input_dim[:3] == (3, 19, 19) and len(cv) == 3 and cv[1] is cv[2] and cv[0].stride[0] == 2 and cv[1].stride[0] == 1:
            return 19
        return None

    def _hip_conv_ok(self, obs_i8):
        return (self.conv_impl == 'gemm' and obs_i8.is_cuda and obs_i8.dtype == torch.int8 and not torch.is_grad_enabled()
                and self._hip_geometry() is not None and self.convs[0].out_channels in (24, 32)
                and self.convs[0].weight.is_contiguous() and self.convs[1].weight.is_contiguous())

    def act_ok(self, obs_i8):
        return (self._hip_conv_ok(obs_i8) and self.mlp1.in_features == 2 + self.n_actions and self.n_actions <= 16
                and self.mlp1.out_features == 10)

    def act_gates(self, obs_i8, last_action_onehot, hidden_state, w_ih_padded=None):
        x = self._front_features_hip(obs_i8, last_action_onehot, padded=True)
        w = self.weight_ih_padded() if w_ih_padded is None else w_ih_padded
        return torch.matmul(x, w.t()), torch.matmul(hidden_state, self.rnn.weight_hh.t())

    def forward_obs(self, obs_i8, last_action_onehot, hidden_state):
        if self._hip_conv_ok(obs_i8) and self.mlp1.in_features == 2 + self.n_actions and self.n_actions <= 16:
            return self.recurrent(self._front_features_hip(obs_i8, last_action_onehot), hidden_state)
        pixel = obs_i8[:, :self.n_pixel].float()
        vec = torch.cat([obs_i8[:, self.n_pixel:].float(), last_action_onehot.float()], dim=1)
        return self.recurrent(self.features_split(pixel, vec), hidden_state)


class RNN(nn.Module):

    def __init__(self, input_shape, args):
        super().__init__()
        self.args = args
        self.fc1 = nn.Linear(input_shape, args.rnn_hidden_dim)
        self.rnn = nn.GRUCell(args.rnn_hidden_dim, args.rnn_hidden_dim)
        self.fc2 = nn.Linear(args.rnn_hidden_dim, args.n_actions)

    def features(self, inputs):
        return f.relu(self.fc1(inputs))

    def recurrent(self, x, hidden_state):
        h = self.rnn(x, hidden_state.reshape(-1, self.args.rnn_hidden_dim))
        return self.fc2(h), h

    def forward(self, obs, hidden_state):
        return self.recurrent(self.features(obs), hidden_state)

    def forward_obs(self, obs_i8, last_action_onehot, hidden_state):
        return self.forward(torch.cat([obs_i8.float(), last_action_onehot.float()], dim=1), hidden_state)
```

Before: 7.472 million.

## Fuse conv9 and MLP-branch backward into one front9 backward kernel

Adds a front9_ops library whose backward kernel computes the conv9 weight gradients and the small direction/action MLP gradients in the same launch and partial-sum buffer, followed by a single reduction. The goal is to remove the separate MLP backward and reduce launches plus the extra pass over obs/x/grad in training. The MLP reduce kernel is also reworked to spread work over output rows with an LDS slab. This adds LDS and partial-buffer pressure and code complexity to the conv backward kernel, and the reduction order changes.

After: 7.527 million (median of 6 runs). Within noise of the previous version (+0.7%).

```diff
diff --git a/__graft_entry__.py b/__graft_entry__.py
--- a/__graft_entry__.py
+++ b/__graft_entry__.py
@@ -31,6 +31,9 @@
         getattr(lib, name)
     lib = _lib.qmix_ops()
     for name in _lib.SIGNATURES['qmix_ops']:
+        getattr(lib, name)
+    lib = _lib.front9_ops()
+    for name in _lib.SIGNATURES['front9_ops']:
         getattr(lib, name)
 
 
diff --git a/include/front9_ops.h b/include/front9_ops.h
--- /dev/null
+++ b/include/front9_ops.h
@@ -0,0 +1,25 @@
+#ifndef FRONT9_OPS_H
+#define FRONT9_OPS_H
+
+#include <stdint.h>
+
+#ifdef __cplusplus
+extern "C" {
+#endif
+
+#define FRONT9_OK 0
+#define FRONT9_ERR_BAD_ARG (-1)
+#define FRONT9_ERR_UNSUPPORTED (-6)
+#define FRONT9_ERR_HIP (-100)
+
+int front9_backward_parts(int od);
+int front9_backward(const int8_t *d_obs, int64_t obs_stride, const int8_t *d_onehot, int n_actions, int64_t rows,
+                    const float *d_x, int64_t x_stride, const float *d_grad_x, int64_t grad_stride, const float *d_w1,
+                    const float *d_b1, const float *d_w2, int od, float *d_part, int n_part, float *d_grads, void *stream);
+int front9_last_hip_error(void);
+
+#ifdef __cplusplus
+}
+#endif
+
+#endif
diff --git a/marl_dmfb_amd/_lib.py b/marl_dmfb_amd/_lib.py
--- a/marl_dmfb_amd/_lib.py
+++ b/marl_dmfb_amd/_lib.py
@@ -177,6 +177,11 @@
                                  vp, vp, vp],
         'qmix_last_hip_error': ([], i32),
     },
+    'front9_ops': {
+        'front9_backward_parts': ([i32], i32),
+        'front9_backward': [vp, i64, vp, i32, i64, vp, i64, vp, i64, vp, vp, vp, i32, vp, i32, vp, vp],
+        'front9_last_hip_error': ([], i32),
+    },
 }
 
 DMFB_VEC_SYMBOLS = list(SIGNATURES['dmfb_vec'])
@@ -205,7 +210,7 @@
 HIP_ERROR = -100
 _LAST_ERROR = {'dmfb_vec_': 'dmfb_vec_last_hip_error', 'meda_vec_': 'meda_vec_last_hip_error', 'crnn_': 'crnn_last_hip_error',
                'gru_': 'gru_last_hip_error', 'rollout_': 'rollout_last_hip_error', 'vdn_': 'vdn_last_hip_error',
-               'qmix_': 'qmix_last_hip_error'}
+               'qmix_': 'qmix_last_hip_error', 'front9_': 'front9_last_hip_error'}
 
 
 def _typed(lib, name):
@@ -278,3 +283,7 @@
 
 def qmix_ops():
     return _library('qmix_ops')
+
+
+def front9_ops():
+    return _library('front9_ops')
diff --git a/marl_dmfb_amd/csrc/conv9_bwd.h b/marl_dmfb_amd/csrc/conv9_bwd.h
--- /dev/null
+++ b/marl_dmfb_amd/csrc/conv9_bwd.h
@@ -0,0 +1,500 @@
+#pragma once
+
+#include <hip/hip_runtime.h>
+
+#include <cstdint>
+
+namespace conv9_bwd {
+
+constexpr int kBlock = 512;
+constexpr int kA1Unit = 100;
+constexpr int kDz1Unit = 108;
+constexpr int kLdsBudget = 158 * 1024;
+constexpr int kMlpOut = 10, kMlpMaxIn = 18;
+constexpr int kMlpItems = kMlpOut * (kMlpMaxIn + 1);
+constexpr int kDirOff = 243;
+
+template <int OD, bool MLP> struct GeoB {
+    static constexpr int DZ2 = 28;
+    static constexpr int DZ_ROW = OD * DZ2 + 4;
+    static constexpr int ROW_FLOATS = (OD / 2) * kA1Unit + OD * DZ2 + 4 + 244 + (OD / 2) * kDz1Unit;
+    static constexpr int FIXED_FLOATS = OD * OD * 9;
+    static constexpr int RBB = ((kLdsBudget / 4 - FIXED_FLOATS) / ROW_FLOATS) < (kBlock / (2 * OD)) ? ((kLdsBudget / 4 - FIXED_FLOATS) / ROW_FLOATS)
+                                                                                                   : (kBlock / (2 * OD));
+    static constexpr size_t LDS_FLOATS = (size_t)FIXED_FLOATS + (size_t)RBB * ROW_FLOATS + OD * 28;
+    static_assert(LDS_FLOATS * 4 <= 160 * 1024, "LDS");
+    static constexpr int UNITS = OD * (OD / 2);
+    static constexpr int NA = UNITS >= kBlock ? kBlock : kBlock / 2;
+    static constexpr int NB = UNITS - NA;
+    static constexpr int XSLICES = NB > 0 ? (kBlock - NA) / NB : 1;
+    static_assert(NB >= 0 && (NB == 0 || (NA + NB * XSLICES <= kBlock && XSLICES <= 8)), "dW2 roles");
+    static constexpr int SPLIT2 = NB > 0 ? 2 : 4, BASE2 = NB > 0 ? kBlock / 2 : 0;
+    static constexpr int END2 = BASE2 + RBB * (OD / 2) * SPLIT2;
+    static_assert(END2 <= kBlock, "P2 roles");
+    static constexpr int FT = kBlock;
+    static constexpr int ITEMS3 = (OD / 2) * 9;
+    static constexpr int RS3 = kBlock / ITEMS3;
+    static constexpr int PART_C = kBlock * 9 + kBlock * 9 + OD + kBlock * 6 + OD;
+    static constexpr int PART = PART_C + (MLP ? kMlpItems : 0);
+    static constexpr int N_CONV = OD * OD * 9 + OD + OD * 27 + OD;
+};
+
+constexpr int kMlpChunk = 64;
+__device__ __noinline__ void mlp_group(const int8_t *__restrict__ obs, long obs_stride, long rows, const float *__restrict__ x,
+                                          long x_stride, const float *__restrict__ g, long g_stride, const int8_t *__restrict__ onehot,
+                                          int n_actions, float *__restrict__ out, int col0, float *lds) {
+    const int nin = 2 + n_actions, n_items = kMlpOut * (nin + 1), tid = threadIdx.x;
+    const long n_groups = min((rows + 255) / 256, 256L);
+    const long b = blockIdx.x;
+    if (b >= n_groups) {
+        for (int i = tid; i < n_items; i += blockDim.x) out[i] = 0.0f;
+        return;
+    }
+    for (int i0 = 0; i0 < n_items; i0 += kMlpChunk) {
+        __syncthreads();
+        if (tid < 256) {
+            for (int i = 0; i < kMlpChunk; ++i) lds[i * 256 + tid] = 0.0f;
+            for (long r = b * 256 + tid; r < rows; r += n_groups * 256) {
+                float gz[kMlpOut], v[kMlpMaxIn + 1];
+#pragma unroll
+                for (int o = 0; o < kMlpOut; ++o) gz[o] = x[r * x_stride + col0 + o] > 0.0f ? g[r * g_stride + col0 + o] : 0.0f;
+                v[0] = (float)obs[r * obs_stride + kDirOff];
+                v[1] = (float)obs[r * obs_stride + kDirOff + 1];
+#pragma unroll
+                for (int k = 2; k <= kMlpMaxIn; ++k) v[k] = k < nin ? (float)onehot[r * n_actions + k - 2] : 0.0f;
+#pragma unroll
+                for (int o = 0; o < kMlpOut; ++o)
+#pragma unroll
+                    for (int k = 0; k <= kMlpMaxIn; ++k) {
+                        if (k > nin) continue;
+                        const int it = o * (nin + 1) + k - i0;
+                        if (it < 0 || it >= kMlpChunk) continue;
+                        float &a = lds[it * 256 + tid];
+                        a = k < nin ? fmaf(gz[o], v[k], a) : a + gz[o];
+                    }
+            }
+        }
+        __syncthreads();
+        const int it = i0 + tid;
+        if (tid < kMlpChunk && it < n_items) {
+            float t = 0.0f;
+            for (int w = 0; w < 4; ++w) {
+                float s[64];
+                const float4 *src = (const float4 *)(lds + tid * 256 + w * 64);
+#pragma unroll
+                for (int j = 0; j < 16; ++j) { const float4 q = src[j]; s[4 * j] = q.x; s[4 * j + 1] = q.y; s[4 * j + 2] = q.z; s[4 * j + 3] = q.w; }
+#pragma unroll
+                for (int d = 32; d > 0; d >>= 1)
+#pragma unroll
+                    for (int l = 0; l < d; ++l) s[l] = s[l] + s[l + d];
+                t += s[0];
+            }
+            out[it] = t;
+        }
+    }
+}
+
+template <int OD, bool MLP>
+__global__ __launch_bounds__(kBlock) void k_conv9_bwd(const int8_t *__restrict__ obs, long obs_stride, long rows,
+                                                      const float *__restrict__ a2, long a2_stride, const float *__restrict__ g, long g_stride,
+                                                      const float *__restrict__ w2, float *__restrict__ part,
+                                                      const float *__restrict__ w1, const float *__restrict__ b1,
+                                                      const int8_t *__restrict__ onehot, int n_actions) {
+    using G = GeoB<OD, MLP>;
+    extern __shared__ __attribute__((aligned(16))) float lds[];
+    float *s_w2 = lds;
+    float *s_a1 = s_w2 + OD * OD * 9;
+    float *s_dz2 = s_a1 + G::RBB * (OD / 2) * kA1Unit;
+    float *s_in = s_dz2 + G::RBB * G::DZ_ROW;
+    float *s_dz1 = s_in + G::RBB * 244;
+    float *s_w1 = s_dz1 + G::RBB * (OD / 2) * kDz1Unit;
+    const int tid = threadIdx.x;
+    for (int i = tid; i < OD * 27; i += kBlock) s_w1[i] = w1[i];
+    if (tid < OD) s_w1[OD * 27 + tid] = b1[tid];
+    for (int i = tid; i < OD * OD * 9; i += kBlock) {
+        const int c2 = i / (OD * 9), rem = i - c2 * OD * 9, c1 = rem / 9, tap = rem - c1 * 9;
+        s_w2[(c2 * 9 + tap) * OD + c1] = w2[i];
+    }
+    float accB2 = 0.0f, accB1 = 0.0f, accB1y = 0.0f;
+    float2 accW2[9], accW1[3];
+#pragma unroll
+    for (int k = 0; k < 9; ++k) accW2[k] = make_float2(0.0f, 0.0f);
+#pragma unroll
+    for (int k = 0; k < 3; ++k) accW1[k] = make_float2(0.0f, 0.0f);
+    const bool pa_full = tid < G::NA;
+    const int pa_unit = pa_full ? tid : G::NA + (G::NB > 0 ? (tid - G::NA) % (G::NB > 0 ? G::NB : 1) : 0);
+    const int pa_slice = pa_full ? 0 : (G::NB > 0 ? (tid - G::NA) / (G::NB > 0 ? G::NB : 1) : 0);
+    const bool pa_on = pa_full || (G::NB > 0 && pa_slice < G::XSLICES);
+    const int pa_step = pa_full ? 1 : G::XSLICES;
+    const int pa_c2 = pa_unit / (OD / 2), pa_cp = pa_unit - pa_c2 * (OD / 2);
+    const int i3 = tid % G::ITEMS3, s3 = tid / G::ITEMS3;
+    const bool p3_on = s3 < G::RS3;
+    const int cp_3 = i3 / 9, c0_3 = (i3 - cp_3 * 9) / 3, kx_3 = i3 - cp_3 * 9 - c0_3 * 3;
+
+    constexpr int kSplit2 = G::SPLIT2, kBase2 = G::BASE2;
+    const int q2 = (tid - kBase2) & (kSplit2 - 1), unit2 = tid >= kBase2 ? (tid - kBase2) / kSplit2 : G::RBB * (OD / 2);
+    const int r2 = unit2 / (OD / 2), cp2 = unit2 - r2 * (OD / 2);
+    const int br = tid / OD, bc = tid - br * OD;
+    const int wave_u = __builtin_amdgcn_readfirstlane(tid >> 6);
+    const bool p2_wave = wave_u * 64 < G::END2 && wave_u * 64 + 64 > kBase2;
+    const bool fetch_wave = wave_u * 64 < G::FT;
+
+    const long n_blocks = (rows + G::RBB - 1) / G::RBB;
+    const long per = (n_blocks + gridDim.x - 1) / gridDim.x;
+    const long blk0 = (long)blockIdx.x * per, blk1 = min(n_blocks, blk0 + per);
+
+    typedef float f32x4 __attribute__((ext_vector_type(4)));
+    const int lane = tid & 63, wave = tid >> 6, j16 = lane & 15, kq = lane >> 4;
+    const int c_nh = (wave >> 1) & 1, c_sub = (wave & 1) + 2 * (wave >> 2), c_ch = c_nh * 16 + j16;
+    const bool c_chv = c_ch < OD;
+    constexpr int NPD = (G::RBB * OD * 25 + G::FT - 1) / G::FT, NPI = (G::RBB * 243 + G::FT - 1) / G::FT, NPW = (NPI + 3) / 4;
+    float pfa[NPD], pfg[NPD];
+    unsigned pfi[NPW];
+#pragma unroll
+    for (int u = 0; u < NPD; ++u) { pfa[u] = 0.0f; pfg[u] = 0.0f; }
+#pragma unroll
+    for (int u = 0; u < NPW; ++u) pfi[u] = 0;
+    auto fetch = [&](long b) {
+        const long r0 = b * G::RBB;
+        const int rvb = b < blk1 ? (int)min((long)G::RBB, rows - r0) : 0;
+        if (rvb <= 0) return;
+        int t_ = tid;
+        asm volatile("" : "+v"(t_));
+#pragma unroll
+        for (int u = 0; u < NPD; ++u) {
+            const int i = min(t_ + u * G::FT, G::RBB * OD * 25 - 1), rr = i / (OD * 25), rem = i - rr * OD * 25;
+            const long row = r0 + min(rr, rvb - 1);
+            pfa[u] = a2[row * a2_stride + rem];
+            pfg[u] = g[row * g_stride + rem];
+        }
+#pragma unroll
+        for (int u = 0; u < NPI; ++u) {
+            const int i = min(t_ + u * G::FT, G::RBB * 243 - 1), rr = i / 243, pp = i - rr * 243;
+            const unsigned byte = (uint8_t)obs[(r0 + min(rr, rvb - 1)) * obs_stride + pp];
+            pfi[u >> 2] = (u & 3) ? (pfi[u >> 2] | byte << (8 * (u & 3))) : byte;
+        }
+    };
+    if (fetch_wave) fetch(blk0);
+    for (long blk = blk0; blk < blk1; ++blk) {
+        const long row0 = blk * G::RBB;
+        const int rv = (int)min((long)G::RBB, rows - row0);
+        __syncthreads();
+        if (fetch_wave) {
+            int t_ = tid;
+            asm volatile("" : "+v"(t_));
+#pragma unroll
+            for (int u = 0; u < NPD; ++u) {
+                const int i = t_ + u * G::FT, rc = i / 25, k = i - rc * 25;
+                if (i < G::RBB * OD * 25) s_dz2[(rc / OD) * G::DZ_ROW + (rc % OD) * G::DZ2 + k] = (rc / OD < rv && pfa[u] > 0.0f) ? pfg[u] : 0.0f;
+            }
+#pragma unroll
+            for (int u = 0; u < NPI; ++u) {
+                const int i = t_ + u * G::FT, rr = i / 243, pp = i - rr * 243;
+                if (i < G::RBB * 243) s_in[rr * 244 + pp] = rr < rv ? (float)(int8_t)(pfi[u >> 2] >> (8 * (u & 3))) : 0.0f;
+            }
+        }
+        __syncthreads();
+        int off1[7], goff[3];
+        float bw1[7];
+        int kq_ = kq, j_ = j16;
+        asm volatile("" : "+v"(kq_), "+v"(j_));
+#pragma unroll
+        for (int s = 0; s < 7; ++s) {
+            const int k = 4 * s + kq_, c0 = k / 9, tap = k - c0 * 9;
+            off1[s] = k < 27 ? c0 * 81 + (tap / 3) * 9 + tap % 3 : 0;
+            const float w = s_w1[(c_chv ? c_ch : 0) * 27 + (k < 27 ? k : 0)];
+            bw1[s] = (c_chv && k < 27) ? w : 0.0f;
+        }
+        const float c_bias = c_chv ? s_w1[OD * 27 + c_ch] : 0.0f;
+#pragma unroll
+        for (int qt = 0; qt < 3; ++qt) { const int p = qt * 16 + j_; goff[qt] = (p / 7) * 9 + p % 7; }
+        for (int rr = c_sub; rr < G::RBB; rr += 4) {
+            float cv[3][7];
+#pragma unroll
+            for (int qt = 0; qt < 3; ++qt)
+#pragma unroll
+                for (int s = 0; s < 7; ++s) cv[qt][s] = s_in[rr * 244 + goff[qt] + off1[s]];
+            f32x4 acc[3];
+#pragma unroll
+            for (int qt = 0; qt < 3; ++qt) acc[qt] = f32x4{c_bias, c_bias, c_bias, c_bias};
+#pragma unroll
+            for (int s = 0; s < 7; ++s)
+#pragma unroll
+                for (int qt = 0; qt < 3; ++qt) acc[qt] = __builtin_amdgcn_mfma_f32_16x16x4f32(cv[qt][s], bw1[s], acc[qt], 0, 0, 0);
+            if (c_chv) {
+                float *dst = s_a1 + (rr * (OD / 2) + (c_ch >> 1)) * kA1Unit + kq * 8 + (c_ch & 1);
+#pragma unroll
+                for (int qt = 0; qt < 3; ++qt)
+#pragma unroll
+                    for (int q = 0; q < 4; ++q) dst[(qt * 16 + q) * 2] = fmaxf(acc[qt][q], 0.0f);
+            }
+        }
+        if (c_sub == 0) {
+            const int rr = j16 < G::RBB ? j16 : G::RBB - 1;
+            f32x4 acc = {c_bias, c_bias, c_bias, c_bias};
+#pragma unroll
+            for (int s = 0; s < 7; ++s) acc = __builtin_amdgcn_mfma_f32_16x16x4f32(s_in[rr * 244 + 60 + off1[s]], bw1[s], acc, 0, 0, 0);
+            if (c_chv) {
+#pragma unroll
+                for (int q = 0; q < 4; ++q)
+                    if (kq * 4 + q < G::RBB) s_a1[((kq * 4 + q) * (OD / 2) + (c_ch >> 1)) * kA1Unit + 96 + (c_ch & 1)] = fmaxf(acc[q], 0.0f);
+            }
+        }
+        __syncthreads();
+        auto unit_rows = [&](int c2, int cp, int r_begin, int r_step) {
+#pragma unroll 1
+            for (int rr = r_begin; rr < rv; rr += r_step) {
+                float dz[G::DZ2];
+                float2 a[kA1Unit / 2];
+                const float4 *pd = (const float4 *)__builtin_assume_aligned(s_dz2 + rr * G::DZ_ROW + c2 * G::DZ2, 16);
+                const float4 *pa = (const float4 *)__builtin_assume_aligned(s_a1 + (size_t)(rr * (OD / 2) + cp) * kA1Unit, 16);
+#pragma unroll
+                for (int j = 0; j < G::DZ2 / 4; ++j) { const float4 t = pd[j]; dz[4 * j] = t.x; dz[4 * j + 1] = t.y; dz[4 * j + 2] = t.z; dz[4 * j + 3] = t.w; }
+#pragma unroll
+                for (int j = 0; j < kA1Unit / 4; ++j) { const float4 t = pa[j]; a[2 * j] = make_float2(t.x, t.y); a[2 * j + 1] = make_float2(t.z, t.w); }
+#pragma unroll
+                for (int kx = 0; kx < 3; ++kx)
+#pragma unroll
+                    for (int ky = 0; ky < 3; ++ky)
+#pragma unroll
+                        for (int x = 0; x < 5; ++x)
+#pragma unroll
+                            for (int y = 0; y < 5; ++y) {
+                                const float z = dz[x * 5 + y];
+                                const float2 v = a[(x + kx) * 7 + y + ky];
+                                accW2[kx * 3 + ky].x = fmaf(z, v.x, accW2[kx * 3 + ky].x);
+                                accW2[kx * 3 + ky].y = fmaf(z, v.y, accW2[kx * 3 + ky].y);
+                            }
+            }
+        };
+        if (tid < G::RBB * OD && br < rv) {
+            const float4 *pd = (const float4 *)__builtin_assume_aligned(s_dz2 + br * G::DZ_ROW + bc * G::DZ2, 16);
+            float t = 0.0f;
+#pragma unroll
+            for (int j = 0; j < 6; ++j) { const float4 v = pd[j]; t += (v.x + v.y) + (v.z + v.w); }
+            accB2 += t + pd[6].x;
+        }
+#ifndef CRNN_PROBE_SKIP_P1
+        if (pa_on) unit_rows(pa_c2, pa_cp, pa_slice, pa_step);
+#endif
+#ifndef CRNN_PROBE_SKIP_P2
+        if (p2_wave) {
+#else
+        if (false) {
+#endif
+            if (unit2 < G::RBB * (OD / 2) && r2 < rv) {
+                float2 da[49];
+#pragma unroll
+                for (int k = 0; k < 49; ++k) da[k] = make_float2(0.0f, 0.0f);
+                const int cbeg = q2 * (OD / kSplit2), cend = cbeg + OD / kSplit2;
+#pragma unroll 1
+                for (int c2 = cbeg; c2 < cend; ++c2) {
+                    float dz[G::DZ2];
+                    float2 w[9];
+                    const float4 *pd = (const float4 *)__builtin_assume_aligned(s_dz2 + r2 * G::DZ_ROW + c2 * G::DZ2, 16);
+#pragma unroll
+                    for (int j = 0; j < G::DZ2 / 4; ++j) { const float4 t = pd[j]; dz[4 * j] = t.x; dz[4 * j + 1] = t.y; dz[4 * j + 2] = t.z; dz[4 * j + 3] = t.w; }
+#pragma unroll
+                    for (int k = 0; k < 9; ++k) w[k] = *(const float2 *)(s_w2 + (c2 * 9 + k) * OD + 2 * cp2);
+#pragma unroll
+                    for (int kx = 0; kx < 3; ++kx)
+#pragma unroll
+                        for (int ky = 0; ky < 3; ++ky)
+#pragma unroll
+                            for (int x = 0; x < 5; ++x)
+#pragma unroll
+                                for (int y = 0; y < 5; ++y) {
+                                    float2 &d = da[(x + kx) * 7 + y + ky];
+                                    const float z = dz[x * 5 + y];
+                                    d.x = fmaf(z, w[kx * 3 + ky].x, d.x);
+                                    d.y = fmaf(z, w[kx * 3 + ky].y, d.y);
+                                }
+                }
+#ifndef CRNN_PROBE_P2_NO_DPP
+#pragma unroll
+                for (int k = 0; k < 49; ++k) {
+                    asm volatile("v_add_f32_dpp %0, %0, %0 quad_perm:[1,0,3,2] row_mask:0xf bank_mask:0xf bound_ctrl:1" : "+v"(da[k].x));
+                    asm volatile("v_add_f32_dpp %0, %0, %0 quad_perm:[1,0,3,2] row_mask:0xf bank_mask:0xf bound_ctrl:1" : "+v"(da[k].y));
+                }
+                if (kSplit2 == 4) {
+                    asm volatile("s_nop 1");
+#pragma unroll
+                    for (int k = 0; k < 49; ++k) {
+                        asm volatile("v_add_f32_dpp %0, %0, %0 quad_perm:[2,3,0,1] row_mask:0xf bank_mask:0xf bound_ctrl:1" : "+v"(da[k].x));
+                        asm volatile("v_add_f32_dpp %0, %0, %0 quad_perm:[2,3,0,1] row_mask:0xf bank_mask:0xf bound_ctrl:1" : "+v"(da[k].y));
+                    }
+                }
+#endif
+#ifdef CRNN_PROBE_P2_NO_MASK
+                if (q2 == 0 && da[0].x == 12345.678f) {
+#else
+                if (q2 == 0) {
+#endif
+                    const float4 *act = (const float4 *)__builtin_assume_aligned(s_a1 + (size_t)unit2 * kA1Unit, 16);
+                    unsigned long long lx = 0, ly = 0;
+#pragma unroll
+                    for (int j = 0; j < 25; ++j) {
+                        const float4 a = act[j];
+                        lx |= (unsigned long long)((a.x > 0.0f ? 1u : 0u) | (a.z > 0.0f ? 2u : 0u)) << (2 * j);
+                        ly |= (unsigned long long)((a.y > 0.0f ? 1u : 0u) | (a.w > 0.0f ? 2u : 0u)) << (2 * j);
+                    }
+                    float4 *dst4 = (float4 *)__builtin_assume_aligned(s_dz1 + (size_t)unit2 * kDz1Unit, 16);
+                    float sx = 0.0f, sy = 0.0f;
+#pragma unroll
+                    for (int j = 0; j < 25; ++j) {
+                        float4 o;
+                        o.x = (lx >> (2 * j)) & 1 ? da[2 * j].x : 0.0f;
+                        o.y = (ly >> (2 * j)) & 1 ? da[2 * j].y : 0.0f;
+                        o.z = (2 * j + 1 < 49 && ((lx >> (2 * j + 1)) & 1)) ? da[2 * j + 1 < 49 ? 2 * j + 1 : 0].x : 0.0f;
+                        o.w = (2 * j + 1 < 49 && ((ly >> (2 * j + 1)) & 1)) ? da[2 * j + 1 < 49 ? 2 * j + 1 : 0].y : 0.0f;
+                        dst4[j] = o;
+                        sx += o.x + o.z;
+                        sy += o.y + o.w;
+                    }
+                    accB1 += sx;
+                    accB1y += sy;
+                }
+            }
+        }
+        if (fetch_wave) fetch(blk + 1);
+        __syncthreads();
+#ifdef CRNN_PROBE_SKIP_P3
+        if (false) {
+#else
+        if (p3_on) {
+#endif
+            for (int rr = s3; rr < rv; rr += G::RS3) {
+                const float2 *pd = (const float2 *)(s_dz1 + (size_t)(rr * (OD / 2) + cp_3) * kDz1Unit);
+                const float *in = s_in + rr * 244 + c0_3 * 81 + kx_3 * 9;
+#pragma unroll
+                for (int x = 0; x < 7; ++x) {
+                    float2 dz[7];
+                    float v[9];
+#pragma unroll
+                    for (int y = 0; y < 7; ++y) dz[y] = pd[x * 7 + y];
+#pragma unroll
+                    for (int y = 0; y < 9; ++y) v[y] = in[x * 9 + y];
+#pragma unroll
+                    for (int ky = 0; ky < 3; ++ky)
+#pragma unroll
+                        for (int y = 0; y < 7; ++y) {
+                            typedef float f32x2 __attribute__((ext_vector_type(2)));
+                            const f32x2 r = __builtin_elementwise_fma((f32x2){dz[y].x, dz[y].y}, (f32x2){v[y + ky], v[y + ky]},
+                                                                      (f32x2){accW1[ky].x, accW1[ky].y});
+                            accW1[ky] = make_float2(r.x, r.y);
+                        }
+                }
+            }
+        }
+    }
+    __syncthreads();
+    if (tid < G::RBB * OD) s_dz2[OD * 16 + bc * 16 + br] = accB2;
+    if (q2 == 0 && unit2 < G::RBB * (OD / 2)) {
+        s_dz2[(2 * cp2) * 16 + r2] = accB1;
+        s_dz2[(2 * cp2 + 1) * 16 + r2] = accB1y;
+    }
+    __syncthreads();
+    float *pp = part + (size_t)blockIdx.x * G::PART;
+#pragma unroll
+    for (int k = 0; k < 9; ++k) { pp[tid * 18 + 2 * k] = accW2[k].x; pp[tid * 18 + 2 * k + 1] = accW2[k].y; }
+    if (tid < OD) {
+        float t = 0.0f;
+        for (int k = 0; k < G::RBB; ++k) t += s_dz2[OD * 16 + tid * 16 + k];
+        pp[kBlock * 18 + tid] = t;
+    }
+#pragma unroll
+    for (int k = 0; k < 3; ++k) { pp[kBlock * 18 + OD + tid * 6 + k] = accW1[k].x; pp[kBlock * 18 + OD + tid * 6 + 3 + k] = accW1[k].y; }
+    if (tid < OD) {
+        float t = 0.0f;
+        for (int k = 0; k < G::RBB; ++k) t += s_dz2[tid * 16 + k];
+        pp[kBlock * 18 + OD + kBlock * 6 + tid] = t;
+    }
+    if (MLP) mlp_group(obs, obs_stride, rows, a2, a2_stride, g, g_stride, onehot, n_actions, pp + G::PART_C, OD * 25, lds);
+}
+
+constexpr int kRedY = 16;
+template <int OD, bool MLP>
+__global__ __launch_bounds__(64 * kRedY) void k_conv9_bwd_reduce(const float *__restrict__ part, int n_part, float *__restrict__ grads, int nin,
+                                                                  int n_groups) {
+    using G = GeoB<OD, MLP>;
+    __shared__ float s_sum[kRedY][64];
+    const int tx = threadIdx.x & 63, ty = threadIdx.x >> 6;
+    constexpr int kConvBlocks = (G::N_CONV + 63) / 64;
+    if (MLP && blockIdx.x >= kConvBlocks) {
+        const int j = (blockIdx.x - kConvBlocks) * 64 + tx, n_w = kMlpOut * nin;
+        const bool on = j < n_w + kMlpOut;
+        const int o = j < n_w ? j / nin : j - n_w, k = j < n_w ? j - o * nin : nin, off = G::PART_C + o * (nin + 1) + k;
+        float t = 0.0f;
+        for (int b0 = 0; b0 < n_groups; b0 += kRedY) {
+            if (on && b0 + ty < n_groups) s_sum[ty][tx] = part[(size_t)(b0 + ty) * G::PART + off];
+            __syncthreads();
+            if (ty == 0 && on)
+                for (int q = 0; q < kRedY && b0 + q < n_groups; ++q) t += s_sum[q][tx];
+            __syncthreads();
+        }
+        if (ty == 0 && on) grads[G::N_CONV + j] = t;
+        return;
+    }
+    const int i = blockIdx.x * 64 + tx;
+    const int n2 = OD * OD * 9, nb = OD, n1 = OD * 27;
+    const int n_out = G::N_CONV;
+    float acc = 0.0f;
+    if (i < n_out) {
+        int off[8], cnt = 0;
+        if (i < n2) {
+            const int pair = i / 9, tap = i - pair * 9, c2 = pair / OD, c1 = pair - c2 * OD;
+            const int unit = c2 * (OD / 2) + (c1 >> 1), comp = 2 * tap + (c1 & 1);
+            if (unit < G::NA) off[cnt++] = unit * 18 + comp;
+            else
+                for (int sl = 0; sl < G::XSLICES && sl < 8; ++sl) off[cnt++] = (G::NA + sl * G::NB + (unit - G::NA)) * 18 + comp;
+        } else if (i < n2 + nb) {
+            off[cnt++] = kBlock * 18 + (i - n2);
+        } else if (i < n2 + nb + n1) {
+            const int jx = i - n2 - nb, c1 = jx / 27, r = jx - c1 * 27, ky = r % 3;
+            const int item = (c1 >> 1) * 9 + r / 3;
+            for (int sl = 0; sl < G::RS3; ++sl) off[cnt++] = kBlock * 18 + OD + (sl * G::ITEMS3 + item) * 6 + (c1 & 1) * 3 + ky;
+        } else {
+            off[cnt++] = kBlock * 18 + OD + kBlock * 6 + (i - n2 - nb - n1);
+        }
+        for (int k = 0; k < cnt; ++k) {
+            float a0 = 0.0f, a1 = 0.0f;
+            int b = ty;
+            for (; b + kRedY < n_part; b += 2 * kRedY) { a0 += part[(size_t)b * G::PART + off[k]]; a1 += part[(size_t)(b + kRedY) * G::PART + off[k]]; }
+            if (b < n_part) a0 += part[(size_t)b * G::PART + off[k]];
+            acc += a0 + a1;
+        }
+    }
+    s_sum[ty][tx] = acc;
+    __syncthreads();
+    if (ty == 0 && i < n_out) {
+        float t = 0.0f;
+#pragma unroll
+        for (int k = 0; k < kRedY; ++k) t += s_sum[k][tx];
+        grads[i] = t;
+    }
+}
+
+template <int OD, bool MLP>
+hipError_t launch(const int8_t *obs, long obs_stride, long rows, const float *x, long x_stride, const float *g, long g_stride,
+                  const float *w2, float *part, int n_part, float *grads, const float *w1, const float *b1, const int8_t *onehot,
+                  int n_actions, hipStream_t s) {
+    using G = GeoB<OD, MLP>;
+    const size_t lds = G::LDS_FLOATS * sizeof(float);
+    static bool raised[64] = {};
+    int dev = 0;
+    (void)hipGetDevice(&dev);
+    if (dev < 0 || dev >= 64 || !raised[dev]) {
+        const hipError_t e = hipFuncSetAttribute((const void *)k_conv9_bwd<OD, MLP>, hipFuncAttributeMaxDynamicSharedMemorySize, (int)lds);
+        if (e != hipSuccess) return e;
+        if (dev >= 0 && dev < 64) raised[dev] = true;
+    }
+    (void)hipGetLastError();
+    hipLaunchKernelGGL((k_conv9_bwd<OD, MLP>), dim3(n_part), dim3(kBlock), lds, s, obs, obs_stride, rows, x, x_stride, g, g_stride,
+                       w2, part, w1, b1, onehot, n_actions);
+    const int n_blocks = (G::N_CONV + 63) / 64 + (MLP ? (kMlpOut * (n_actions + 3) + 63) / 64 : 0);
+    const int n_groups = (int)((rows + 255) / 256 < 256 ? (rows + 255) / 256 : 256);
+    hipLaunchKernelGGL((k_conv9_bwd_reduce<OD, MLP>), dim3(n_blocks), dim3(64 * kRedY), 0, s, part, n_part, grads, 2 + n_actions, n_groups);
+    return hipGetLastError();
+}
+
+}
diff --git a/marl_dmfb_amd/csrc/crnn_ops.hip b/marl_dmfb_amd/csrc/crnn_ops.hip
--- a/marl_dmfb_amd/csrc/crnn_ops.hip
+++ b/marl_dmfb_amd/csrc/crnn_ops.hip
@@ -12,385 +12,9 @@
 #include "crnn_mfma.h"
 #include "crnn_mfma19.h"
 #include "crnn_bwd19.h"
+#include "conv9_bwd.h"
 
 namespace {
-
-constexpr int kBlock = 512;
-constexpr int kA1Stride = 52;
-constexpr int kDz1Unit = 108;
-
-constexpr int kLdsBudget = 158 * 1024;
-
-template <int OD> struct GeoB {
-    static constexpr int DZ2 = 28;
-    static constexpr int DZ_ROW = OD * DZ2 + 4;
-    static constexpr int ROW_FLOATS = OD * kA1Stride + OD * DZ2 + 4 + 244 + (OD / 2) * kDz1Unit;
-    static constexpr int FIXED_FLOATS = OD * OD * 9;
-    static constexpr int RBB = ((kLdsBudget / 4 - FIXED_FLOATS) / ROW_FLOATS) < (kBlock / (2 * OD)) ? ((kLdsBudget / 4 - FIXED_FLOATS) / ROW_FLOATS)
-                                                                                                   : (kBlock / (2 * OD));
-    static constexpr size_t LDS_FLOATS = (size_t)FIXED_FLOATS + (size_t)RBB * ROW_FLOATS + OD * 28;
-    static constexpr int UNITS = OD * (OD / 2);
-    static constexpr int NA = UNITS >= kBlock ? kBlock : kBlock / 2;
-    static constexpr int NB = UNITS - NA;
-    static constexpr int XSLICES = NB > 0 ? (kBlock - NA) / NB : 1;
-    static_assert(NB >= 0 && (NB == 0 || (NA + NB * XSLICES <= kBlock && XSLICES <= 8)), "dW2 roles");
-    static constexpr int ITEMS3 = (OD / 2) * 9;
-    static constexpr int RS3 = kBlock / ITEMS3;
-    static constexpr int PART = kBlock * 9 + kBlock * 9 + OD + kBlock * 6 + OD;
-};
-
-template <int OD>
-__global__ __launch_bounds__(kBlock) void k_conv9_bwd(const int8_t *__restrict__ obs, long obs_stride, long rows,
-                                                      const float *__restrict__ a2, long a2_stride, const float *__restrict__ g, long g_stride,
-                                                      const float *__restrict__ w2, float *__restrict__ part,
-                                                      const float *__restrict__ w1, const float *__restrict__ b1) {
-    using G = GeoB<OD>;
-    extern __shared__ __attribute__((aligned(16))) float lds[];
-    float *s_w2 = lds;
-    float *s_a1 = s_w2 + OD * OD * 9;
-    float *s_dz2 = s_a1 + G::RBB * OD * kA1Stride;
-    float *s_in = s_dz2 + G::RBB * G::DZ_ROW;
-    float *s_dz1 = s_in + G::RBB * 244;
-    float *s_w1 = s_dz1 + G::RBB * (OD / 2) * kDz1Unit;
-    const int tid = threadIdx.x;
-    for (int i = tid; i < OD * 27; i += kBlock) s_w1[i] = w1[i];
-    if (tid < OD) s_w1[OD * 27 + tid] = b1[tid];
-    for (int i = tid; i < OD * OD * 9; i += kBlock) {
-        const int c2 = i / (OD * 9), rem = i - c2 * OD * 9, c1 = rem / 9, tap = rem - c1 * 9;
-        s_w2[(c2 * 9 + tap) * OD + c1] = w2[i];
-    }
-    float accB2 = 0.0f, accB1 = 0.0f, accB1y = 0.0f;
-    float2 accW2[9], accW1[3];
-#pragma unroll
-    for (int k = 0; k < 9; ++k) accW2[k] = make_float2(0.0f, 0.0f);
-#pragma unroll
-    for (int k = 0; k < 3; ++k) accW1[k] = make_float2(0.0f, 0.0f);
-    const bool pa_full = tid < G::NA;
-    const int pa_unit = pa_full ? tid : G::NA + (G::NB > 0 ? (tid - G::NA) % (G::NB > 0 ? G::NB : 1) : 0);
-    const int pa_slice = pa_full ? 0 : (G::NB > 0 ? (tid - G::NA) / (G::NB > 0 ? G::NB : 1) : 0);
-    const bool pa_on = pa_full || (G::NB > 0 && pa_slice < G::XSLICES);
-    const int pa_step = pa_full ? 1 : G::XSLICES;
-    const int pa_c2 = pa_unit / (OD / 2), pa_cp = pa_unit - pa_c2 * (OD / 2);
-    const int i3 = tid % G::ITEMS3, s3 = tid / G::ITEMS3;
-    const bool p3_on = s3 < G::RS3;
-    const int cp_3 = i3 / 9, c0_3 = (i3 - cp_3 * 9) / 3, kx_3 = i3 - cp_3 * 9 - c0_3 * 3;
-
-    constexpr int kSplit2 = G::NB > 0 ? 2 : 4, kBase2 = G::NB > 0 ? kBlock / 2 : 0;
-    const int q2 = (tid - kBase2) & (kSplit2 - 1), unit2 = tid >= kBase2 ? (tid - kBase2) / kSplit2 : G::RBB * (OD / 2);
-    const int r2 = unit2 / (OD / 2), cp2 = unit2 - r2 * (OD / 2);
-    const int br = tid / OD, bc = tid - br * OD;
-
-    const long n_blocks = (rows + G::RBB - 1) / G::RBB;
-    const long per = (n_blocks + gridDim.x - 1) / gridDim.x;
-    const long blk0 = (long)blockIdx.x * per, blk1 = min(n_blocks, blk0 + per);
-
-    typedef float f32x4 __attribute__((ext_vector_type(4)));
-    const int lane = tid & 63, wave = tid >> 6, j16 = lane & 15, kq = lane >> 4;
-    const int c_nh = (wave >> 1) & 1, c_sub = (wave & 1) + 2 * (wave >> 2), c_ch = c_nh * 16 + j16;
-    const bool c_chv = c_ch < OD;
-    constexpr int NPD = (G::RBB * OD * 25 + kBlock - 1) / kBlock, NPI = (G::RBB * 243 + kBlock - 1) / kBlock;
-    float pfa[NPD], pfg[NPD];
-    int pfi[NPI];
-#pragma unroll
-    for (int u = 0; u < NPD; ++u) { pfa[u] = 0.0f; pfg[u] = 0.0f; }
-#pragma unroll
-    for (int u = 0; u < NPI; ++u) pfi[u] = 0;
-    auto fetch = [&](long b) {
-        const long r0 = b * G::RBB;
-        const int rvb = b < blk1 ? (int)min((long)G::RBB, rows - r0) : 0;
-        if (rvb <= 0) return;
-        int t_ = tid;
-        asm volatile("" : "+v"(t_));
-#pragma unroll
-        for (int u = 0; u < NPD; ++u) {
-            const int i = min(t_ + u * kBlock, G::RBB * OD * 25 - 1), rr = i / (OD * 25), rem = i - rr * OD * 25;
-            const long row = r0 + min(rr, rvb - 1);
-            pfa[u] = a2[row * a2_stride + rem];
-            pfg[u] = g[row * g_stride + rem];
-        }
-#pragma unroll
-        for (int u = 0; u < NPI; ++u) {
-            const int i = min(t_ + u * kBlock, G::RBB * 243 - 1), rr = i / 243, pp = i - rr * 243;
-            pfi[u] = obs[(r0 + min(rr, rvb - 1)) * obs_stride + pp];
-        }
-    };
-    fetch(blk0);
-    for (long blk = blk0; blk < blk1; ++blk) {
-        const long row0 = blk * G::RBB;
-        const int rv = (int)min((long)G::RBB, rows - row0);
-        __syncthreads();
-        int t_ = tid;
-        asm volatile("" : "+v"(t_));
-#pragma unroll
-        for (int u = 0; u < NPD; ++u) {
-            const int i = t_ + u * kBlock, rc = i / 25, k = i - rc * 25;
-            if (i < G::RBB * OD * 25) s_dz2[(rc / OD) * G::DZ_ROW + (rc % OD) * G::DZ2 + k] = (rc / OD < rv && pfa[u] > 0.0f) ? pfg[u] : 0.0f;
-        }
-#pragma unroll
-        for (int u = 0; u < NPI; ++u) {
-            const int i = t_ + u * kBlock, rr = i / 243, pp = i - rr * 243;
-            if (i < G::RBB * 243) s_in[rr * 244 + pp] = rr < rv ? (float)pfi[u] : 0.0f;
-        }
-        __syncthreads();
-        int off1[7], goff[3];
-        float bw1[7];
-        int kq_ = kq, j_ = j16;
-        asm volatile("" : "+v"(kq_), "+v"(j_));
-#pragma unroll
-        for (int s = 0; s < 7; ++s) {
-            const int k = 4 * s + kq_, c0 = k / 9, tap = k - c0 * 9;
-            off1[s] = k < 27 ? c0 * 81 + (tap / 3) * 9 + tap % 3 : 0;
-            const float w = s_w1[(c_chv ? c_ch : 0) * 27 + (k < 27 ? k : 0)];
-            bw1[s] = (c_chv && k < 27) ? w : 0.0f;
-        }
-        const float c_bias = c_chv ? s_w1[OD * 27 + c_ch] : 0.0f;
-#pragma unroll
-        for (int qt = 0; qt < 3; ++qt) { const int p = qt * 16 + j_; goff[qt] = (p / 7) * 9 + p % 7; }
-        for (int rr = c_sub; rr < G::RBB; rr += 4) {
-            float cv[3][7];
-#pragma unroll
-            for (int qt = 0; qt < 3; ++qt)
-#pragma unroll
-                for (int s = 0; s < 7; ++s) cv[qt][s] = s_in[rr * 244 + goff[qt] + off1[s]];
-            f32x4 acc[3];
-#pragma unroll
-            for (int qt = 0; qt < 3; ++qt) acc[qt] = f32x4{c_bias, c_bias, c_bias, c_bias};
-#pragma unroll
-            for (int s = 0; s < 7; ++s)
-#pragma unroll
-                for (int qt = 0; qt < 3; ++qt) acc[qt] = __builtin_amdgcn_mfma_f32_16x16x4f32(cv[qt][s], bw1[s], acc[qt], 0, 0, 0);
-            if (c_chv) {
-                float *dst = s_a1 + ((rr * (OD / 2) + (c_ch >> 1)) * kA1Stride + kq * 4) * 2 + (c_ch & 1);
-#pragma unroll
-                for (int qt = 0; qt < 3; ++qt)
-#pragma unroll
-                    for (int q = 0; q < 4; ++q) dst[(qt * 16 + q) * 2] = fmaxf(acc[qt][q], 0.0f);
-            }
-        }
-        if (c_sub == 0) {
-            const int rr = j16 < G::RBB ? j16 : G::RBB - 1;
-            f32x4 acc = {c_bias, c_bias, c_bias, c_bias};
-#pragma unroll
-            for (int s = 0; s < 7; ++s) acc = __builtin_amdgcn_mfma_f32_16x16x4f32(s_in[rr * 244 + 60 + off1[s]], bw1[s], acc, 0, 0, 0);
-            if (c_chv) {
-#pragma unroll
-                for (int q = 0; q < 4; ++q)
-                    if (kq * 4 + q < G::RBB) s_a1[(((kq * 4 + q) * (OD / 2) + (c_ch >> 1)) * kA1Stride + 48) * 2 + (c_ch & 1)] = fmaxf(acc[q], 0.0f);
-            }
-        }
-        __syncthreads();
-        auto unit_rows = [&](int c2, int cp, int r_begin, int r_step) {
-#pragma unroll 1
-            for (int rr = r_begin; rr < rv; rr += r_step) {
-                float dz[G::DZ2];
-                float2 a[kA1Stride];
-                const float4 *pd = (const float4 *)__builtin_assume_aligned(s_dz2 + rr * G::DZ_ROW + c2 * G::DZ2, 16);
-                const float4 *pa = (const float4 *)__builtin_assume_aligned(s_a1 + (size_t)(rr * (OD / 2) + cp) * 2 * kA1Stride, 16);
-#pragma unroll
-                for (int j = 0; j < G::DZ2 / 4; ++j) { const float4 t = pd[j]; dz[4 * j] = t.x; dz[4 * j + 1] = t.y; dz[4 * j + 2] = t.z; dz[4 * j + 3] = t.w; }
-#pragma unroll
-                for (int j = 0; j < kA1Stride / 2; ++j) { const float4 t = pa[j]; a[2 * j] = make_float2(t.x, t.y); a[2 * j + 1] = make_float2(t.z, t.w); }
-#pragma unroll
-                for (int kx = 0; kx < 3; ++kx)
-#pragma unroll
-                    for (int ky = 0; ky < 3; ++ky)
-#pragma unroll
-                        for (int x = 0; x < 5; ++x)
-#pragma unroll
-                            for (int y = 0; y < 5; ++y) {
-                                const float z = dz[x * 5 + y];
-                                const float2 v = a[(x + kx) * 7 + y + ky];
-                                accW2[kx * 3 + ky].x = fmaf(z, v.x, accW2[kx * 3 + ky].x);
-                                accW2[kx * 3 + ky].y = fmaf(z, v.y, accW2[kx * 3 + ky].y);
-                            }
-            }
-        };
-        if (tid < G::RBB * OD && br < rv) {
-            const float4 *pd = (const float4 *)__builtin_assume_aligned(s_dz2 + br * G::DZ_ROW + bc * G::DZ2, 16);
-            float t = 0.0f;
-#pragma unroll
-            for (int j = 0; j < 6; ++j) { const float4 v = pd[j]; t += (v.x + v.y) + (v.z + v.w); }
-            accB2 += t + pd[6].x;
-        }
-#ifndef CRNN_PROBE_SKIP_P1
-        if (pa_on) unit_rows(pa_c2, pa_cp, pa_slice, pa_step);
-#endif
-#ifndef CRNN_PROBE_SKIP_P2
-        const bool p2 = unit2 < G::RBB * (OD / 2) && r2 < rv;
-#else
-        const bool p2 = false;
-#endif
-        if (p2) {
-            float2 da[49];
-#pragma unroll
-            for (int k = 0; k < 49; ++k) da[k] = make_float2(0.0f, 0.0f);
-            const int cbeg = q2 * (OD / kSplit2), cend = cbeg + OD / kSplit2;
-#pragma unroll 1
-            for (int c2 = cbeg; c2 < cend; ++c2) {
-                float dz[G::DZ2];
-                float2 w[9];
-                const float4 *pd = (const float4 *)__builtin_assume_aligned(s_dz2 + r2 * G::DZ_ROW + c2 * G::DZ2, 16);
-#pragma unroll
-                for (int j = 0; j < G::DZ2 / 4; ++j) { const float4 t = pd[j]; dz[4 * j] = t.x; dz[4 * j + 1] = t.y; dz[4 * j + 2] = t.z; dz[4 * j + 3] = t.w; }
-#pragma unroll
-                for (int k = 0; k < 9; ++k) w[k] = *(const float2 *)(s_w2 + (c2 * 9 + k) * OD + 2 * cp2);
-#pragma unroll
-                for (int kx = 0; kx < 3; ++kx)
-#pragma unroll
-                    for (int ky = 0; ky < 3; ++ky)
-#pragma unroll
-                        for (int x = 0; x < 5; ++x)
-#pragma unroll
-                            for (int y = 0; y < 5; ++y) {
-                                float2 &d = da[(x + kx) * 7 + y + ky];
-                                const float z = dz[x * 5 + y];
-                                d.x = fmaf(z, w[kx * 3 + ky].x, d.x);
-                                d.y = fmaf(z, w[kx * 3 + ky].y, d.y);
-                            }
-            }
-#ifndef CRNN_PROBE_P2_NO_DPP
-#pragma unroll
-            for (int k = 0; k < 49; ++k) {
-                asm volatile("v_add_f32_dpp %0, %0, %0 quad_perm:[1,0,3,2] row_mask:0xf bank_mask:0xf bound_ctrl:1" : "+v"(da[k].x));
-                asm volatile("v_add_f32_dpp %0, %0, %0 quad_perm:[1,0,3,2] row_mask:0xf bank_mask:0xf bound_ctrl:1" : "+v"(da[k].y));
-            }
-            if (kSplit2 == 4) {
-                asm volatile("s_nop 1");
-#pragma unroll
-                for (int k = 0; k < 49; ++k) {
-                    asm volatile("v_add_f32_dpp %0, %0, %0 quad_perm:[2,3,0,1] row_mask:0xf bank_mask:0xf bound_ctrl:1" : "+v"(da[k].x));
-                    asm volatile("v_add_f32_dpp %0, %0, %0 quad_perm:[2,3,0,1] row_mask:0xf bank_mask:0xf bound_ctrl:1" : "+v"(da[k].y));
-                }
-            }
-#endif
-#ifdef CRNN_PROBE_P2_NO_MASK
-            if (q2 == 0 && da[0].x == 12345.678f) {
-#else
-            if (q2 == 0) {
-#endif
-                const float4 *act = (const float4 *)__builtin_assume_aligned(s_a1 + (size_t)unit2 * 2 * kA1Stride, 16);
-                unsigned long long lx = 0, ly = 0;
-#pragma unroll
-                for (int j = 0; j < 25; ++j) {
-                    const float4 a = act[j];
-                    lx |= (unsigned long long)((a.x > 0.0f ? 1u : 0u) | (a.z > 0.0f ? 2u : 0u)) << (2 * j);
-                    ly |= (unsigned long long)((a.y > 0.0f ? 1u : 0u) | (a.w > 0.0f ? 2u : 0u)) << (2 * j);
-                }
-                float4 *dst4 = (float4 *)__builtin_assume_aligned(s_dz1 + (size_t)unit2 * kDz1Unit, 16);
-                float sx = 0.0f, sy = 0.0f;
-#pragma unroll
-                for (int j = 0; j < 25; ++j) {
-                    float4 o;
-                    o.x = (lx >> (2 * j)) & 1 ? da[2 * j].x : 0.0f;
-                    o.y = (ly >> (2 * j)) & 1 ? da[2 * j].y : 0.0f;
-                    o.z = (2 * j + 1 < 49 && ((lx >> (2 * j + 1)) & 1)) ? da[2 * j + 1 < 49 ? 2 * j + 1 : 0].x : 0.0f;
-                    o.w = (2 * j + 1 < 49 && ((ly >> (2 * j + 1)) & 1)) ? da[2 * j + 1 < 49 ? 2 * j + 1 : 0].y : 0.0f;
-                    dst4[j] = o;
-                    sx += o.x + o.z;
-                    sy += o.y + o.w;
-                }
-                accB1 += sx;
-                accB1y += sy;
-            }
-        }
-        __syncthreads();
-        fetch(blk + 1);
-#ifdef CRNN_PROBE_SKIP_P3
-        if (false) {
-#else
-        if (p3_on) {
-#endif
-            for (int rr = s3; rr < rv; rr += G::RS3) {
-                const float2 *pd = (const float2 *)(s_dz1 + (size_t)(rr * (OD / 2) + cp_3) * kDz1Unit);
-                const float *in = s_in + rr * 244 + c0_3 * 81 + kx_3 * 9;
-#pragma unroll
-                for (int x = 0; x < 7; ++x) {
-                    float2 dz[7];
-                    float v[9];
-#pragma unroll
-                    for (int y = 0; y < 7; ++y) dz[y] = pd[x * 7 + y];
-#pragma unroll
-                    for (int y = 0; y < 9; ++y) v[y] = in[x * 9 + y];
-#pragma unroll
-                    for (int ky = 0; ky < 3; ++ky)
-#pragma unroll
-                        for (int y = 0; y < 7; ++y) {
-                            typedef float f32x2 __attribute__((ext_vector_type(2)));
-                            const f32x2 r = __builtin_elementwise_fma((f32x2){dz[y].x, dz[y].y}, (f32x2){v[y + ky], v[y + ky]},
-                                                                      (f32x2){accW1[ky].x, accW1[ky].y});
-                            accW1[ky] = make_float2(r.x, r.y);
-                        }
-                }
-            }
-        }
-    }
-    __syncthreads();
-    if (tid < G::RBB * OD) s_dz2[OD * 16 + bc * 16 + br] = accB2;
-    if (q2 == 0 && unit2 < G::RBB * (OD / 2)) {
-        s_dz2[(2 * cp2) * 16 + r2] = accB1;
-        s_dz2[(2 * cp2 + 1) * 16 + r2] = accB1y;
-    }
-    __syncthreads();
-    float *pp = part + (size_t)blockIdx.x * G::PART;
-#pragma unroll
-    for (int k = 0; k < 9; ++k) { pp[tid * 18 + 2 * k] = accW2[k].x; pp[tid * 18 + 2 * k + 1] = accW2[k].y; }
-    if (tid < OD) {
-        float t = 0.0f;
-        for (int k = 0; k < G::RBB; ++k) t += s_dz2[OD * 16 + tid * 16 + k];
-        pp[kBlock * 18 + tid] = t;
-    }
-#pragma unroll
-    for (int k = 0; k < 3; ++k) { pp[kBlock * 18 + OD + tid * 6 + k] = accW1[k].x; pp[kBlock * 18 + OD + tid * 6 + 3 + k] = accW1[k].y; }
-    if (tid < OD) {
-        float t = 0.0f;
-        for (int k = 0; k < G::RBB; ++k) t += s_dz2[tid * 16 + k];
-        pp[kBlock * 18 + OD + kBlock * 6 + tid] = t;
-    }
-}
-
-constexpr int kRedY = 16;
-template <int OD>
-__global__ __launch_bounds__(64 * kRedY) void k_conv9_bwd_reduce(const float *__restrict__ part, int n_part, float *__restrict__ grads) {
-    using G = GeoB<OD>;
-    __shared__ float s_sum[kRedY][64];
-    const int tx = threadIdx.x & 63, ty = threadIdx.x >> 6;
-    const int i = blockIdx.x * 64 + tx;
-    const int n2 = OD * OD * 9, nb = OD, n1 = OD * 27;
-    float acc = 0.0f;
-    if (i < n2 + nb + n1 + nb) {
-        int off[8], cnt = 0;
-        if (i < n2) {
-            const int pair = i / 9, tap = i - pair * 9, c2 = pair / OD, c1 = pair - c2 * OD;
-            const int unit = c2 * (OD / 2) + (c1 >> 1), comp = 2 * tap + (c1 & 1);
-            if (unit < G::NA) off[cnt++] = unit * 18 + comp;
-            else
-                for (int sl = 0; sl < G::XSLICES && sl < 8; ++sl) off[cnt++] = (G::NA + sl * G::NB + (unit - G::NA)) * 18 + comp;
-        } else if (i < n2 + nb) {
-            off[cnt++] = kBlock * 18 + (i - n2);
-        } else if (i < n2 + nb + n1) {
-            const int jx = i - n2 - nb, c1 = jx / 27, r = jx - c1 * 27, ky = r % 3;
-            const int item = (c1 >> 1) * 9 + r / 3;
-            for (int sl = 0; sl < G::RS3; ++sl) off[cnt++] = kBlock * 18 + OD + (sl * G::ITEMS3 + item) * 6 + (c1 & 1) * 3 + ky;
-        } else {
-            off[cnt++] = kBlock * 18 + OD + kBlock * 6 + (i - n2 - nb - n1);
-        }
-        for (int k = 0; k < cnt; ++k) {
-            float a0 = 0.0f, a1 = 0.0f;
-            int b = ty;
-            for (; b + kRedY < n_part; b += 2 * kRedY) { a0 += part[(size_t)b * G::PART + off[k]]; a1 += part[(size_t)(b + kRedY) * G::PART + off[k]]; }
-            if (b < n_part) a0 += part[(size_t)b * G::PART + off[k]];
-            acc += a0 + a1;
-        }
-    }
-    s_sum[ty][tx] = acc;
-    __syncthreads();
-    if (ty == 0 && i < n2 + nb + n1 + nb) {
-        float t = 0.0f;
-#pragma unroll
-        for (int k = 0; k < kRedY; ++k) t += s_sum[k][tx];
-        grads[i] = t;
-    }
-}
 
 constexpr int kMlpBlock = 256, kMlpOut = 10, kMlpMaxIn = 18, kMlpMaxParts = 256;
 __global__ __launch_bounds__(kMlpBlock) void k_mlp_bwd(const int8_t *__restrict__ obs, long obs_stride, int dir_off,
@@ -434,14 +58,22 @@
         part[(size_t)blockIdx.x * kMlpOut * (kMlpMaxIn + 1) + i] = t;
     }
 }
-__global__ __launch_bounds__(256) void k_mlp_bwd_reduce(const float *__restrict__ part, int n_part, int nin, float *__restrict__ dw, float *__restrict__ db) {
-    const int i = threadIdx.x;
-    if (i >= kMlpOut * nin + kMlpOut) return;
-    const int o = i < kMlpOut * nin ? i / nin : i - kMlpOut * nin, k = i < kMlpOut * nin ? i - o * nin : kMlpMaxIn;
+constexpr int kMlpRedY = 8;
+__global__ __launch_bounds__(32 * kMlpRedY) void k_mlp_bwd_reduce(const float *__restrict__ part, int n_part, int nin, float *__restrict__ dw, float *__restrict__ db) {
+    __shared__ float s_slab[kMlpRedY][32];
+    const int o = blockIdx.x, k = threadIdx.x & 31, ty = threadIdx.x >> 5;
+    const bool on = k <= nin;
+    const int kk = k < nin ? k : kMlpMaxIn;
     float t = 0.0f;
-    for (int b = 0; b < n_part; ++b) t += part[(size_t)b * kMlpOut * (kMlpMaxIn + 1) + o * (kMlpMaxIn + 1) + k];
-    if (i < kMlpOut * nin) dw[i] = t;
-    else db[o] = t;
+    for (int b0 = 0; b0 < n_part; b0 += kMlpRedY) {
+        if (on && b0 + ty < n_part) s_slab[ty][k] = part[(size_t)(b0 + ty) * kMlpOut * (kMlpMaxIn + 1) + o * (kMlpMaxIn + 1) + kk];
+        __syncthreads();
+        if (ty == 0 && on)
+            for (int q = 0; q < kMlpRedY && b0 + q < n_part; ++q) t += s_slab[q][k];
+        __syncthreads();
+    }
+    if (ty == 0 && k < nin) dw[o * nin + k] = t;
+    if (ty == 0 && k == nin) db[o] = t;
 }
 
 struct LiveRows { const int32_t *chips; const int32_t *n; int rows_per_chip; };
@@ -487,16 +119,7 @@
 int launch_bwd(const int8_t *obs, long obs_stride, long rows, const float *a2, long a2_stride,
                const float *g, long g_stride, const float *w2, float *part, int grid, float *grads, const float *w1, const float *b1,
                hipStream_t s) {
-    using G = GeoB<OD>;
-    const size_t lds = G::LDS_FLOATS * sizeof(float);
-    static LdsLimit lds_limit;
-    if (const int rc = lds_limit.raise((const void *)k_conv9_bwd<OD>, lds)) return rc;
-    HIP_TRY(launch_status([&] {
-        hipLaunchKernelGGL((k_conv9_bwd<OD>), dim3(grid), dim3(kBlock), lds, s, obs, obs_stride, rows, a2, a2_stride, g, g_stride,
-                           w2, part, w1, b1);
-        const int n_out = OD * OD * 9 + OD + OD * 27 + OD;
-        hipLaunchKernelGGL((k_conv9_bwd_reduce<OD>), dim3((n_out + 63) / 64), dim3(64 * kRedY), 0, s, part, grid, grads);
-    }));
+    HIP_TRY((conv9_bwd::launch<OD, false>(obs, obs_stride, rows, a2, a2_stride, g, g_stride, w2, part, grid, grads, w1, b1, nullptr, 0, s)));
     return CRNN_OK;
 }
 
@@ -577,7 +200,9 @@
     return launch19<32>(d_obs, obs_stride, rows, d_w1, d_b1, d_w3, d_b3, d_out, out_stride, out_cols, d_onehot, n_actions, d_mlp_w, d_mlp_b, (hipStream_t)stream);
 }
 
-int crnn_conv9_backward_parts(int od) { return od == 24 ? GeoB<24>::PART : od == 32 ? GeoB<32>::PART : CRNN_ERR_UNSUPPORTED; }
+int crnn_conv9_backward_parts(int od) {
+    return od == 24 ? conv9_bwd::GeoB<24, false>::PART : od == 32 ? conv9_bwd::GeoB<32, false>::PART : CRNN_ERR_UNSUPPORTED;
+}
 
 int crnn_conv9_backward(const int8_t *d_obs, int64_t obs_stride, int64_t rows, const float *d_out, int64_t out_stride,
                         const float *d_grad_out, int64_t grad_stride, const float *d_w1, const float *d_b1, const float *d_w2,
@@ -603,7 +228,7 @@
     HIP_TRY(launch_status([&] {
         hipLaunchKernelGGL(k_mlp_bwd, dim3(grid), dim3(kMlpBlock), 0, (hipStream_t)stream, d_obs, (long)obs_stride, dir_offset, d_onehot, n_actions,
                            (long)rows, d_out, (long)out_stride, d_grad_out, (long)grad_stride, col0, d_part);
-        hipLaunchKernelGGL(k_mlp_bwd_reduce, dim3(1), dim3(256), 0, (hipStream_t)stream, d_part, grid, 2 + n_actions, d_grad_w, d_grad_b);
+        hipLaunchKernelGGL(k_mlp_bwd_reduce, dim3(kMlpOut), dim3(32 * kMlpRedY), 0, (hipStream_t)stream, d_part, grid, 2 + n_actions, d_grad_w, d_grad_b);
     }));
     return CRNN_OK;
 }
diff --git a/marl_dmfb_amd/csrc/front9_ops.hip b/marl_dmfb_amd/csrc/front9_ops.hip
--- /dev/null
+++ b/marl_dmfb_amd/csrc/front9_ops.hip
@@ -0,0 +1,39 @@
+#include <hip/hip_runtime.h>
+
+#include <cstdint>
+
+#include "../../include/front9_ops.h"
+
+#define HIP_ABI_TAG "front9_ops"
+#define HIP_ABI_ERR FRONT9_ERR_HIP
+#include "hip_abi.h"
+#include "conv9_bwd.h"
+
+extern "C" {
+
+int front9_backward_parts(int od) {
+    return od == 24 ? conv9_bwd::GeoB<24, true>::PART : od == 32 ? conv9_bwd::GeoB<32, true>::PART : FRONT9_ERR_UNSUPPORTED;
+}
+
+int front9_backward(const int8_t *d_obs, int64_t obs_stride, const int8_t *d_onehot, int n_actions, int64_t rows,
+                    const float *d_x, int64_t x_stride, const float *d_grad_x, int64_t grad_stride, const float *d_w1,
+                    const float *d_b1, const float *d_w2, int od, float *d_part, int n_part, float *d_grads, void *stream) {
+    if (!d_obs || !d_x || !d_grad_x || !d_w1 || !d_b1 || !d_w2 || !d_part || !d_grads || (n_actions > 0 && !d_onehot) || rows <= 0 ||
+        n_actions < 0 || n_actions > 16 || n_part < 1 || n_part > 256 || obs_stride < conv9_bwd::kDirOff + 2)
+        return FRONT9_ERR_BAD_ARG;
+    if (od != 24 && od != 32) return FRONT9_ERR_UNSUPPORTED;
+    if (x_stride < od * 25 + 10 || grad_stride < od * 25 + 10) return FRONT9_ERR_BAD_ARG;
+    if (n_part < (rows + 255) / 256 && n_part < 256) return FRONT9_ERR_BAD_ARG;
+    const hipStream_t s = (hipStream_t)stream;
+    if (od == 24)
+        HIP_TRY((conv9_bwd::launch<24, true>(d_obs, obs_stride, rows, d_x, x_stride, d_grad_x, grad_stride, d_w2, d_part, n_part, d_grads,
+                                            d_w1, d_b1, d_onehot, n_actions, s)));
+    else
+        HIP_TRY((conv9_bwd::launch<32, true>(d_obs, obs_stride, rows, d_x, x_stride, d_grad_x, grad_stride, d_w2, d_part, n_part, d_grads,
+                                            d_w1, d_b1, d_onehot, n_actions, s)));
+    return FRONT9_OK;
+}
+
+int front9_last_hip_error(void) { return g_last_hip; }
+
+}
diff --git a/marl_dmfb_amd/network/base_net.py b/marl_dmfb_amd/network/base_net.py
--- a/marl_dmfb_amd/network/base_net.py
+++ b/marl_dmfb_amd/network/base_net.py
@@ -62,6 +62,20 @@
     return g_w, g_b
 
 
+def _front9_backward(obs_i8, onehot_i8, x, g, w1c, b1c, w2c, od):
+    from .. import _lib
+    lib = _lib.checked('front9_ops')
+    if g.stride(1) != 1:
+        g = g.contiguous()
+    R, A = obs_i8.shape[0], onehot_i8.shape[1]
+    tot = torch.empty(od * od * 9 + od + od * 27 + od + 10 * (2 + A) + 10, dtype=torch.float32, device=g.device)
+    part = torch.empty((N_PART, lib.front9_backward_parts(od)), dtype=torch.float32, device=g.device)
+    lib.front9_backward(obs_i8.data_ptr(), obs_i8.stride(0), onehot_i8.data_ptr(), A, R, x.data_ptr(), x.stride(0), g.data_ptr(),
+                        g.stride(0), w1c.data_ptr(), b1c.data_ptr(), w2c.data_ptr(), od, part.data_ptr(), N_PART, tot.data_ptr(),
+                        torch.cuda.current_stream(g.device).cuda_stream)
+    return tot
+
+
 class _ConvFront9(torch.autograd.Function):
 
     @staticmethod
@@ -113,10 +127,10 @@
         (s1, s2) = ctx.shapes
         od = s1[0]
         n2 = od * od * 9
-        tot = _conv9_backward(obs_i8, x, g, w1c, b1c, w2c, od)
-        g_mw, g_mb = _mlp_branch_backward(obs_i8, 243, onehot_i8, x, g, od * 25)
-        return (None, None, tot[n2 + od:n2 + od + od * 27].view(s1), tot[n2 + od + od * 27:], tot[:n2].view(s2), tot[n2:n2 + od],
-                g_mw, g_mb, None)
+        tot = _front9_backward(obs_i8, onehot_i8, x, g, w1c, b1c, w2c, od)
+        nc, A = n2 + od + od * 27 + od, onehot_i8.shape[1]
+        return (None, None, tot[n2 + od:n2 + od + od * 27].view(s1), tot[n2 + od + od * 27:nc], tot[:n2].view(s2), tot[n2:n2 + od],
+                tot[nc:nc + 10 * (2 + A)].view(10, 2 + A), tot[nc + 10 * (2 + A):], None)
 
 
 class _Front19Train(torch.autograd.Function):
```
